# scroll-tech/halo2-snark-aggregator

Hardware: AMD Instinct MI355X
Metric: BN254 G1 MSM points/sec (higher is better)
Workload: dtype u32 (9 x 29-bit limbs, Montgomery R = 2^261; 254-bit prime-field integers)

## Files before the change

### halo2-snark-aggregator_amd/__init__.py

```python
from __future__ import annotations

import ctypes as C
import os
from typing import List, Optional, Sequence

_HERE = os.path.dirname(os.path.abspath(__file__))
LIB_PATH = os.path.join(_HERE, "libh2agg.so")
HEADER_PATH = os.path.join(os.path.dirname(_HERE), "include", "h2agg.h")

OK, ERR_INVALID, ERR_DIV_ZERO, ERR_EMPTY, ERR_HIP, ERR_NONCANONICAL, ERR_NOMEM, ERR_BAD_POINT, ERR_PEER, ERR_NOT_IN_TABLE = range(10)
OP_ADD, OP_SUB, OP_MUL, OP_SQR, OP_INV, OP_DIV = range(6)
FR_FFT_LOCAL = 10
FR_FFT_MAX_K = 24
FR_POLY_CHUNK = 11
FR_SCAN_CHUNK = 11
FR_PROD_MAX_COLUMNS = 16
FR_SORT_TILE = 11
FR_SORT_TILE_MIN = 4
FR_COMPRESS_MAX_COLUMNS = 1 << 16
EXPR_MAX_DEPTH = 16

IDENTITY_JAC = (0).to_bytes(32, "little") + (1).to_bytes(32, "little") + (0).to_bytes(32, "little")


# ... 21 lines not shown
def load_library():
    global _lib
    if _lib is not None:
        return _lib
    if not os.path.exists(LIB_PATH):
        raise ImportError(
            "libh2agg.so is not built (%s). Run `python __graft_entry__.py build` — the HIP extension is "
            "required, there is no CPU fallback." % LIB_PATH)
    try:
        import torch
    except ImportError:
        pass
    lib = C.CDLL(LIB_PATH)
    u8p, vp, sz, i32, u64 = C.c_char_p, C.c_void_p, C.c_size_t, C.c_int, C.c_uint64
    ctxp = C.c_void_p
    protos = {
        "h2agg_create": (i32, [i32, C.POINTER(ctxp)]),
        "h2agg_destroy": (None, [ctxp]),
        "h2agg_last_error": (C.c_char_p, [ctxp]),
        "h2agg_set_stream": (i32, [ctxp, vp]),
        "h2agg_synchronize": (i32, [ctxp]),
        "h2agg_describe": (C.c_char_p, [ctxp]),
        "h2agg_fr_batch_op": (i32, [ctxp, i32, u8p, u8p, sz, vp]),
        "h2agg_fr_batch_pow_constant": (i32, [ctxp, u8p, sz, u64, vp]),
        "h2agg_fr_tape_eval": (i32, [ctxp, u8p, sz, vp, sz, vp, sz, vp]),
        "h2agg_fr_mul_add_accumulate": (i32, [ctxp, u8p, sz, u8p, vp]),
        "h2agg_fr_sum_with_coeff_and_constant": (i32, [ctxp, u8p, u8p, sz, u8p, vp]),
        "h2agg_g1_batch_add": (i32, [ctxp, u8p, u8p, sz, i32, vp]),
        "h2agg_g1_batch_scalar_mul": (i32, [ctxp, u8p, u8p, sz, vp]),
        "h2agg_g1_batch_to_affine": (i32, [ctxp, u8p, sz, vp]),
        "h2agg_g1_sum": (i32, [ctxp, u8p, sz, vp]),
        "h2agg_g1_batch_decompress": (i32, [ctxp, u8p, sz, vp, vp]),
        "h2agg_g1_batch_compress": (i32, [ctxp, u8p, sz, vp]),
        "h2agg_g1_msm": (i32, [ctxp, vp, vp, sz, vp]),
        "h2agg_g1_msm_jac": (i32, [ctxp, vp, vp, sz, vp]),
        "h2agg_g1_msm_segmented": (i32, [ctxp, vp, vp, sz, C.POINTER(u64), sz, vp]),
        "h2agg_host_alloc": (i32, [ctxp, sz, C.POINTER(vp)]),
        "h2agg_host_free": (i32, [ctxp, vp]),
        "h2agg_eval_flat": (i32, [ctxp, u8p, u8p, u8p, sz, vp]),
        "h2agg_bases_upload": (i32, [ctxp, u8p, sz, C.POINTER(u64)]),
        "h2agg_bases_generate": (i32, [ctxp, vp, sz, C.POINTER(u64)]),
        "h2agg_bases_precompute": (i32, [ctxp, u64, i32]),
        "h2agg_bases_download": (i32, [ctxp, u64, sz, sz, vp]),
        "h2agg_bases_free": (i32, [ctxp, u64]),
        "h2agg_g1_msm_preloaded": (i32, [ctxp, u64, u8p, sz, vp]),
        "h2agg_instance_commitment": (i32, [ctxp, u64, u8p, sz, sz, vp]),
        "h2agg_g1_msm_device": (i32, [ctxp, u64, vp, sz, vp]),
        "h2agg_g1_msm_device_async": (i32, [ctxp, u64, vp, sz, vp]),
        "h2agg_schema_create": (i32, [ctxp, C.POINTER(C.c_void_p)]),
        "h2agg_schema_destroy": (None, [C.c_void_p]),
        "h2agg_schema_node_commitment": (i32, [C.c_void_p, C.c_char_p, u8p, C.POINTER(C.c_uint32)]),
        "h2agg_schema_node_eval": (i32, [C.c_void_p, u8p, C.POINTER(C.c_uint32)]),
        "h2agg_schema_node_scalar": (i32, [C.c_void_p, u8p, C.POINTER(C.c_uint32)]),
        "h2agg_schema_node_add": (i32, [C.c_void_p, C.c_uint32, C.c_uint32, C.POINTER(C.c_uint32)]),
        "h2agg_schema_node_mul": (i32, [C.c_void_p, C.c_uint32, C.c_uint32, C.POINTER(C.c_uint32)]),
        "h2agg_schema_estimate": (i32, [C.c_void_p, C.c_uint32, C.POINTER(C.c_size_t)]),
        "h2agg_schema_evaluation_queries": (i32, [C.c_void_p, sz, C.POINTER(C.c_char_p), u8p, u8p,
                                                  C.POINTER(C.c_uint32)]),
        "h2agg_schema_batch_multi_open": (i32, [C.c_void_p, C.c_char_p, sz, C.POINTER(C.c_int32), u8p,
                                                C.POINTER(C.c_uint32), sz, u8p, u8p, u8p,
                                                C.POINTER(C.c_uint32), C.POINTER(C.c_uint32)]),
        "h2agg_schema_eval": (i32, [C.c_void_p, C.c_uint32, vp, C.POINTER(i32), vp]),
        "h2agg_evaluate_multiopen_proof": (i32, [C.c_void_p, C.c_uint32, C.c_uint32, vp, vp]),
        "h2agg_evaluate_multiopen_prepare": (i32, [C.c_void_p, C.c_uint32, C.c_uint32]),
        "h2agg_schema_name_count": (C.c_size_t, [C.c_void_p]),
        "h2agg_schema_name": (C.c_char_p, [C.c_void_p, C.c_size_t]),
        "h2agg_g1_msm_device_batch_async": (C.c_int, [C.c_void_p, C.c_uint64, C.c_void_p, C.c_size_t, C.c_size_t, C.c_void_p]),
        "h2agg_schema_query_set_commitment": (C.c_int, [C.c_void_p, C.c_uint32, C.c_char_p]),
        "h2agg_g1_batch_to_affine_device": (C.c_int, [C.c_void_p, C.c_void_p, C.c_size_t, C.c_char_p]),
        "h2agg_schema_names_joined": (C.c_size_t, [C.c_void_p, C.c_char_p, C.c_size_t]),
        "h2agg_schema_point_list_len": (C.c_size_t, [C.c_void_p]),
        "h2agg_poseidon_squeeze_batch": (i32, [ctxp, u8p, sz, sz, C.POINTER(C.c_uint32), sz, vp]),
        "h2agg_transcript_read_batch": (i32, [ctxp, u8p, sz, sz, C.c_char_p, sz, u8p, sz, u8p, sz, vp, vp]),
        "h2agg_vk_create": (i32, [ctxp, u8p, sz, C.POINTER(C.c_void_p)]),
        "h2agg_vk_set_transcript": (i32, [C.c_void_p, i32]),
        "h2agg_hash_transcript_read_batch": (i32, [ctxp, i32, u8p, sz, sz, C.c_char_p, sz, u8p, sz, u8p, sz, vp, vp]),
        "h2agg_hash_transcript_read_batch_host": (i32, [i32, u8p, sz, sz, C.c_char_p, sz, u8p, sz, u8p, sz, vp, vp, i32]),
        "h2agg_hash_digest_host": (i32, [i32, u8p, sz, vp]),
        "h2agg_vk_destroy": (None, [C.c_void_p]),
        "h2agg_verify_aggregation": (i32, [ctxp, vp, sz, u8p, u8p, vp, vp, vp, C.POINTER(i32)]),
        "h2agg_verify_aggregation_ex": (i32, [ctxp, vp, sz, u8p, u8p, vp, vp, vp, C.POINTER(i32), vp, sz]),
        "h2agg_verify_aggregation_sharded": (i32, [ctxp, vp, sz, vp, u8p, u8p, vp, vp, vp, C.POINTER(i32), vp, sz]),
        "h2agg_debug_configure": (i32, [ctxp, C.c_char_p, i32]),
        "h2agg_verify_proofs": (i32, [ctxp, vp, sz, u8p, u8p, vp, vp, C.POINTER(C.c_int32), C.POINTER(i32), vp, sz]),
        "h2agg_verify_plan_stats": (i32, [ctxp, C.POINTER(C.c_uint64), C.POINTER(C.c_uint64), C.POINTER(C.c_uint64)]),
        "h2agg_last_phases": (C.c_char_p, [ctxp]),
        "h2agg_transcript_configure": (i32, [ctxp, i32]),
        "h2agg_poseidon_squeeze_batch_host": (i32, [u8p, sz, sz, C.POINTER(C.c_uint32), sz, vp, i32]),
        "h2agg_host_threads": (i32, []),
        "h2agg_host_sponge_kind": (i32, []),
        "h2agg_comm_unique_id": (i32, [vp]),
        "h2agg_comm_init_rank": (i32, [ctxp, u8p, i32, i32]),
        "h2agg_comm_create": (i32, [C.POINTER(i32), i32, C.POINTER(ctxp)]),
        "h2agg_comm_size": (i32, [ctxp]),
        "h2agg_comm_rank": (i32, [ctxp]),
        "h2agg_comm_last_error": (C.c_char_p, []),
        "h2agg_allgather_add_points": (i32, [C.POINTER(ctxp), i32, u8p, sz, vp]),
        "h2agg_pairing_check": (i32, [ctxp, u8p, u8p, sz, C.POINTER(i32)]),
        "h2agg_g2_batch_decompress": (i32, [ctxp, u8p, sz, vp]),
        "h2agg_bases_fft": (i32, [ctxp, u64, C.c_uint, i32, C.POINTER(u64)]),
        "h2agg_params_setup": (i32, [ctxp, C.c_uint, u8p, C.POINTER(u64), C.POINTER(u64)]),
        "h2agg_fr_fft": (i32, [ctxp, vp, C.c_uint, i32, u8p, vp]),
        "h2agg_fr_fft_device": (i32, [ctxp, vp, C.c_uint, i32, u8p, vp]),
        "h2agg_fr_poly_eval": (i32, [ctxp, vp, sz, C.c_uint, C.POINTER(C.c_uint32), sz, u8p, sz, vp]),
        "h2agg_fr_poly_eval_device": (i32, [ctxp, vp, sz, C.c_uint, C.POINTER(C.c_uint32), sz, u8p, sz, vp]),
        "h2agg_fr_poly_divide": (i32, [ctxp, vp, C.c_uint, u8p, vp, vp]),
        "h2agg_fr_poly_divide_device": (i32, [ctxp, vp, C.c_uint, u8p, vp, vp]),
        "h2agg_kzg_multiopen": (i32, [ctxp, u64, vp, sz, C.c_uint, C.POINTER(C.c_uint32), sz, u8p, sz, u8p, vp,
                                      C.POINTER(C.c_uint32), C.POINTER(sz)]),
        "h2agg_kzg_multiopen_device": (i32, [ctxp, u64, vp, sz, C.c_uint, C.POINTER(C.c_uint32), sz, u8p, sz, u8p, vp,
                                             C.POINTER(C.c_uint32), C.POINTER(sz)]),
        "h2agg_fr_batch_invert": (i32, [ctxp, vp, sz, vp]),
        "h2agg_fr_batch_invert_device": (i32, [ctxp, vp, sz, vp]),
        "h2agg_fr_grand_product": (i32, [ctxp, vp, vp, C.c_uint, sz, u8p, vp, vp]),
        "h2agg_fr_grand_product_device": (i32, [ctxp, vp, vp, C.c_uint, sz, u8p, vp, vp]),
        "h2agg_permutation_product": (i32, [ctxp, vp, vp, sz, C.c_uint, sz, u8p, u8p, u8p, u8p, u8p, vp, vp]),
        "h2agg_permutation_product_device": (i32, [ctxp, vp, vp, sz, C.c_uint, sz, u8p, u8p, u8p, u8p, u8p, vp, vp]),
        "h2agg_lookup_product": (i32, [ctxp, vp, vp, vp, vp, C.c_uint, sz, u8p, u8p, vp, vp]),
        "h2agg_lookup_product_device": (i32, [ctxp, vp, vp, vp, vp, C.c_uint, sz, u8p, u8p, vp, vp]),
        "h2agg_lookup_permute": (i32, [ctxp, vp, vp, C.c_uint, sz, vp, vp]),
        "h2agg_lookup_permute_device": (i32, [ctxp, vp, vp, C.c_uint, sz, vp, vp]),
        "h2agg_fr_columns_compress": (i32, [ctxp, vp, sz, C.c_uint, u8p, vp]),
        "h2agg_fr_columns_compress_device": (i32, [ctxp, vp, sz, C.c_uint, u8p, vp]),
        "h2agg_vk_expressions_eval": (i32, [ctxp, vp, i32, sz, C.c_uint, vp, vp, vp, u8p, u8p, vp]),
        "h2agg_vk_expressions_eval_device": (i32, [ctxp, vp, i32, sz, C.c_uint, vp, vp, vp, u8p, u8p, vp]),
        "h2agg_quotient": (i32, [ctxp, vp, vp, vp, vp, vp, vp, vp, vp, vp, u8p, u8p, u8p, u8p, u8p, u8p, vp]),
        "h2agg_quotient_device": (i32, [ctxp, vp, vp, vp, vp, vp, vp, vp, vp, vp, u8p, u8p, u8p, u8p, u8p, u8p, vp]),
        "h2agg_g2_scalar_mul": (i32, [u8p, u8p, vp]),
        "h2agg_g2_batch_compress": (i32, [u8p, sz, vp]),
        "h2agg_pairing_product": (i32, [ctxp, u8p, u8p, sz, vp]),
        "h2agg_final_pair_check": (i32, [ctxp, u8p, u8p, u8p, u8p, C.POINTER(i32)]),
        "h2agg_msm_configure": (i32, [ctxp, i32, i32, i32]),
        "h2agg_msm_configure_glv": (i32, [ctxp, i32]),
        "h2agg_msm_configure_lanes_per_bucket": (i32, [ctxp, i32]),
        "h2agg_msm_configure_sort": (i32, [ctxp, i32, i32]),
        "h2agg_msm_set_tail_overlap": (i32, [ctxp, i32]),
        "h2agg_profile_enable": (i32, [ctxp, i32]),
        "h2agg_profile_reset": (i32, [ctxp]),
        "h2agg_profile_stage_count": (i32, [ctxp]),
        "h2agg_profile_stage_name": (C.c_char_p, [ctxp, i32]),
        "h2agg_profile_stage_get": (i32, [ctxp, i32, C.POINTER(C.c_double), C.POINTER(u64)]),
    }
    for name, (res, args) in protos.items():
        fn = getattr(lib, name)
        fn.restype = res
        fn.argtypes = args
    lib._h2agg_protos = tuple(protos)
    _lib = lib
    return lib


def exported_symbols() -> Sequence[str]:
    return load_library()._h2agg_protos


def _need(buf, nbytes: int, what: str):
    if buf is None or len(buf) != nbytes:
        raise ValueError("%s must be exactly %d bytes (got %s)" % (what, nbytes, "None" if buf is None else len(buf)))


def _check_host(rc: int, what: str):
    if rc == ERR_BAD_POINT:
        raise BadPoint(rc, what + ": invalid G2 point")
    if rc != OK:
        raise H2AggError(rc, what + (": input integer >= modulus" if rc == ERR_NONCANONICAL else " failed"))

# ... 548 lines not shown
        self._check(self._lib.h2agg_hash_transcript_read_batch(self._ctx, *args, pts, ch))
        nproofs = len(proofs)
        return ([pts.raw[64 * npts * i:64 * npts * (i + 1)] for i in range(nproofs)],
                [ch.raw[32 * nsq * i:32 * nsq * (i + 1)] for i in range(nproofs)])

    @staticmethod
    def comm_unique_id() -> bytes:
        out = C.create_string_buffer(128)
        rc = load_library().h2agg_comm_unique_id(out)
        if rc != OK:
            why = load_library().h2agg_comm_last_error() or b""
            raise H2AggError(rc, "h2agg_comm_unique_id failed: " + (why.decode(errors="replace") or "RCCL error"))
        return out.raw

    def comm_init_rank(self, unique_id: bytes, rank: int, nranks: int):
        _need(unique_id, 128, "unique_id")
        self._check(self._lib.h2agg_comm_init_rank(self._ctx, unique_id, rank, nranks))

    def comm_size(self) -> int:
        return self._lib.h2agg_comm_size(self._ctx)

    def comm_rank(self) -> int:
        return self._lib.h2agg_comm_rank(self._ctx)

    def allgather_add_points(self, partial_jac: bytes) -> bytes:
        npts = len(partial_jac) // 96
        _need(partial_jac, 96 * npts, "partial_jac")
        out = C.create_string_buffer(max(64 * npts, 1))
        arr = (C.c_void_p * 1)(self._ctx)
        self._check(self._lib.h2agg_allgather_add_points(arr, 1, partial_jac, npts, out))
        return out.raw[:64 * npts]

    def pairing_check(self, g1_aff: bytes, g2_aff: bytes) -> bool:
        n = len(g1_aff) // 64
        _need(g1_aff, 64 * n, "g1_aff")
        _need(g2_aff, 128 * n, "g2_aff")
        ok = C.c_int()
        self._check(self._lib.h2agg_pairing_check(self._ctx, g1_aff, g2_aff, n, C.byref(ok)))
        return bool(ok.value)

    def pairing_product(self, g1_aff: bytes, g2_aff: bytes) -> bytes:
        n = len(g1_aff) // 64
        _need(g1_aff, 64 * n, "g1_aff")
        _need(g2_aff, 128 * n, "g2_aff")
        out = C.create_string_buffer(384)
        self._check(self._lib.h2agg_pairing_product(self._ctx, g1_aff, g2_aff, n, out))
        return out.raw

    def g2_batch_decompress(self, data: bytes) -> bytes:
        n = len(data) // 64
        _need(data, 64 * n, "data")
        out = C.create_string_buffer(max(128 * n, 1))
        self._check(self._lib.h2agg_g2_batch_decompress(self._ctx, data, n, out))
        return out.raw[:128 * n]

    def final_pair_check(self, left_aff: bytes, right_aff: bytes, s_g2: bytes, g2: bytes) -> bool:
        _need(left_aff, 64, "left_aff")
        _need(right_aff, 64, "right_aff")
        _need(s_g2, 128, "s_g2")
        _need(g2, 128, "g2")
        ok = C.c_int()
        self._check(self._lib.h2agg_final_pair_check(self._ctx, left_aff, right_aff, s_g2, g2, C.byref(ok)))
        return bool(ok.value)

    def g1_msm_device_batch_async(self, handle: int, d_scalars_ptr: int, n: int, batch: int, d_out_ptr: int):
        self._check(self._lib.h2agg_g1_msm_device_batch_async(self._ctx, handle, C.c_void_p(d_scalars_ptr), n, batch,
                                                              C.c_void_p(d_out_ptr)))

    def msm_configure(self, window_bits: int = 0, reduce_segment: int = 0, big_bucket_threshold: int = 0):
        self._check(self._lib.h2agg_msm_configure(self._ctx, window_bits, reduce_segment, big_bucket_threshold))

    def msm_configure_glv(self, mode: int = 0):
        self._check(self._lib.h2agg_msm_configure_glv(self._ctx, mode))

    def msm_configure_lanes_per_bucket(self, lanes: int = 0):
        self._check(self._lib.h2agg_msm_configure_lanes_per_bucket(self._ctx, lanes))

    def msm_configure_sort(self, sub_bits: int = 0, tile: int = 0):
        self._check(self._lib.h2agg_msm_configure_sort(self._ctx, sub_bits, tile))

    def debug_configure(self, key: str, value: int):
        self._check(self._lib.h2agg_debug_configure(self._ctx, key.encode(), int(value)))

    def msm_set_tail_overlap(self, level: int = 2):
        self._check(self._lib.h2agg_msm_set_tail_overlap(self._ctx, int(level)))

    def profile_enable(self, on=True, only_stage: Optional[int] = None):
        mode = (2 + int(only_stage)) if (on and only_stage is not None) else int(bool(on))
        self._check(self._lib.h2agg_profile_enable(self._ctx, mode))

    def profile_reset(self):
        self._check(self._lib.h2agg_profile_reset(self._ctx))

    def profile_stages(self):
        out = {}
        for i in range(self._lib.h2agg_profile_stage_count(self._ctx)):
            ms, cnt = C.c_double(), C.c_uint64()
            self._check(self._lib.h2agg_profile_stage_get(self._ctx, i, C.byref(ms), C.byref(cnt)))
            out[self._lib.h2agg_profile_stage_name(self._ctx, i).decode()] = (ms.value, cnt.value)
        return out


def host_sponge_kind() -> str:
    return "ifma" if load_library().h2agg_host_sponge_kind() == 1 else "scalar"


def poseidon_squeeze_batch_host(elems: bytes, nproofs: int, upto: Sequence[int], max_threads: int = 0,
                                kernel: Optional[str] = None) -> bytes:
    lib = load_library()
    max_threads = (max_threads & 0xffff) | {None: 0, "scalar": 0x10000, "ifma": 0x20000}[kernel]
    nelem = (len(elems) // 32) // max(nproofs, 1)
    _need(elems, 32 * nelem * nproofs, "elems")
    nsq = len(upto)
    arr = (C.c_uint32 * max(nsq, 1))(*upto)
    out = C.create_string_buffer(32 * max(nproofs * nsq, 1))
    rc = lib.h2agg_poseidon_squeeze_batch_host(elems, nproofs, nelem, arr, nsq, out, max_threads)
    if rc != OK:
        raise H2AggError(rc, "h2agg_poseidon_squeeze_batch_host: " + ("element >= r" if rc == ERR_NONCANONICAL else "invalid arguments"))
    return out.raw[:32 * nproofs * nsq]


TRANSCRIPT_KINDS = {"poseidon": 0, "sha256": 1, "keccak256": 2}


def _hash_transcript_args(kind, proofs, script, consts, ext_points_aff):
    nproofs = len(proofs)
    plen = 64 * script.count("P") + 32 * script.count("S")
    for p in proofs:
        _need(p, plen, "proof")
    npts, nsq, nx = script.count("P"), script.count("Q"), script.count("X")
    _need(consts, 32 * script.count("C"), "consts")
    _need(ext_points_aff, 64 * nx * nproofs, "ext_points_aff")
    pts = C.create_string_buffer(max(64 * npts * nproofs, 1))
    ch = C.create_string_buffer(max(32 * nsq * nproofs, 1))
    sb = script.encode()
    k = TRANSCRIPT_KINDS.get(kind, kind)
    return (k, b"".join(proofs), plen, nproofs, sb, len(sb), consts, len(consts) // 32, ext_points_aff, nx), pts, ch, npts, nsq


def hash_transcript_read_batch_host(kind: str, proofs: Sequence[bytes], script: str, consts: bytes = b"",
                                    ext_points_aff: bytes = b"", max_threads: int = 0):
    args, pts, ch, npts, nsq = _hash_transcript_args(kind, proofs, script, consts, ext_points_aff)
    rc = load_library().h2agg_hash_transcript_read_batch_host(*args, pts, ch, max_threads)
    if rc != OK:
        what = {ERR_BAD_POINT: "invalid point encoding in proof", ERR_NONCANONICAL: "invalid field element encoding in proof"}
        raise (BadPoint if rc == ERR_BAD_POINT else H2AggError)(rc, "h2agg_hash_transcript_read_batch_host: " + what.get(rc, "invalid arguments"))
    nproofs = len(proofs)
    return ([pts.raw[64 * npts * i:64 * npts * (i + 1)] for i in range(nproofs)],
            [ch.raw[32 * nsq * i:32 * nsq * (i + 1)] for i in range(nproofs)])


def hash_digest_host(kind: str, msg: bytes) -> bytes:
    out = C.create_string_buffer(32)
    rc = load_library().h2agg_hash_digest_host(TRANSCRIPT_KINDS.get(kind, kind), msg, len(msg), out)
    if rc != OK:
        raise H2AggError(rc, "h2agg_hash_digest_host: invalid arguments")
    return out.raw


def host_threads() -> int:
    return load_library().h2agg_host_threads()


class H2AggGroup:

    def __init__(self, devices: Sequence[int]):
# ... 156 lines not shown
```

### halo2-snark-aggregator_amd/csrc/batch_kernels.hpp

```cpp
#pragma once
#include "g1.hpp"

namespace h2agg {

enum : uint32_t { FLAG_NONCANONICAL = 1u, FLAG_DIV_ZERO = 2u, FLAG_BAD_POINT = 4u };

constexpr int BLOCK = 256;

__global__ void k_flags_roll(uint32_t* flags) {
    flags[2] |= flags[0];
    flags[0] = 0;
}

template <int NLIMB>
FP_INLINE void lds_put(uint32_t* lds, int tid, const uint32_t* v) {
#pragma unroll
    for (int k = 0; k < NLIMB; ++k) lds[k * BLOCK + tid] = v[k];
}
template <int NLIMB>
FP_INLINE void lds_get(const uint32_t* lds, int tid, uint32_t* v) {
#pragma unroll
    for (int k = 0; k < NLIMB; ++k) v[k] = lds[k * BLOCK + tid];
}
constexpr int XYZZ_WORDS = 4 * NL;
FP_INLINE void lds_put_xyzz(uint32_t* lds, int tid, const G1XYZZ& p) {
    lds_put<NL>(lds, tid, p.x.l);
    lds_put<NL>(lds + NL * BLOCK, tid, p.y.l);
    lds_put<NL>(lds + 2 * NL * BLOCK, tid, p.zz.l);
    lds_put<NL>(lds + 3 * NL * BLOCK, tid, p.zzz.l);
}
FP_INLINE G1XYZZ lds_get_xyzz(const uint32_t* lds, int tid) {
    G1XYZZ p;
    lds_get<NL>(lds, tid, p.x.l);
    lds_get<NL>(lds + NL * BLOCK, tid, p.y.l);
    lds_get<NL>(lds + 2 * NL * BLOCK, tid, p.zz.l);
    lds_get<NL>(lds + 3 * NL * BLOCK, tid, p.zzz.l);
    return p;
}
__device__ __noinline__ G1XYZZ block_sum_xyzz(G1XYZZ v, uint32_t* lds) {
    const int tid = threadIdx.x;
    lds_put_xyzz(lds, tid, v);
    __syncthreads();
#pragma unroll 1
    for (int s = BLOCK / 2; s >= 1; s >>= 1) {
        if (tid < s) {
            G1XYZZ o = lds_get_xyzz(lds, tid + s);
            v = xyzz_add(v, o);
            lds_put_xyzz(lds, tid, v);
        }
        __syncthreads();
    }
    return v;
}
__device__ __noinline__ Fr block_sum_fr(Fr v, uint32_t* lds) {
    const int tid = threadIdx.x;
    lds_put<NL>(lds, tid, v.l);
    __syncthreads();
#pragma unroll 1
    for (int s = BLOCK / 2; s >= 1; s >>= 1) {
        if (tid < s) {
            Fr o;
            lds_get<NL>(lds, tid + s, o.l);
            v = fp_cond_sub<FrParams>(fp_add<FrParams>(v, o));
            lds_put<NL>(lds, tid, v.l);
        }
        __syncthreads();
    }
    return v;
}

__global__ void __launch_bounds__(BLOCK) k_fr_batch_op(int op, const uint8_t* __restrict__ a,
                                                       const uint8_t* __restrict__ b, size_t n,
                                                       uint8_t* __restrict__ out, uint32_t* flags) {
    for (size_t i = (size_t)blockIdx.x * BLOCK + threadIdx.x; i < n; i += (size_t)gridDim.x * BLOCK) {
        Fr x = fp_load<FrParams>(a + 32 * i);
        uint32_t bad = !fp_is_canonical<FrParams>(x);
        Fr y = Fr::zero();
        if (op <= 2 || op == 5) {
            y = fp_load<FrParams>(b + 32 * i);
            bad |= !fp_is_canonical<FrParams>(y);
        }
        if (bad) atomicOr(flags, FLAG_NONCANONICAL);
        Fr z;
        switch (op) {
        case 0: z = fp_cond_sub<FrParams>(fp_add<FrParams>(x, y)); break;
        case 1: z = fp_cond_sub<FrParams>(fp_sub<1, FrParams>(x, y)); break;
        case 2: z = fp_cond_sub<FrParams>(fp_mul<FrParams>(fp_to_mont<FrParams>(x), y)); break;
        case 3: z = fp_cond_sub<FrParams>(fp_mul<FrParams>(fp_to_mont<FrParams>(x), x)); break;
        case 5:
            if (y.is_zero_int()) atomicOr(flags, FLAG_DIV_ZERO);
            z = fp_cond_sub<FrParams>(fp_mul<FrParams>(fp_inv<FrParams>(fp_to_mont<FrParams>(y)), x));
            break;
        default:
            if (x.is_zero_int()) atomicOr(flags, FLAG_DIV_ZERO);
            z = fp_from_mont<FrParams>(fp_inv<FrParams>(fp_to_mont<FrParams>(x)));
// ... 124 lines not shown
__device__ __noinline__ G1XYZZ g1_scalar_mul(const G1Affine& base, const U256& s) {
    G1XYZZ acc = G1XYZZ::identity();
    U256 k = s;
#pragma unroll 1
    for (int it = 0; it < 256; ++it) {
        acc = xyzz_double(acc);
        const uint32_t top = k.w[7] >> 31;
#pragma unroll
        for (int i = 7; i > 0; --i) k.w[i] = (k.w[i] << 1) | (k.w[i - 1] >> 31);
        k.w[0] <<= 1;
        if (top) xyzz_add_affine(acc, base);
    }
    return acc;
}

__global__ void __launch_bounds__(BLOCK) k_g1_batch_scalar_mul(const uint8_t* __restrict__ bases,
                                                               const uint8_t* __restrict__ scalars, size_t n,
                                                               uint8_t* __restrict__ out, uint32_t* flags) {
    for (size_t i = (size_t)blockIdx.x * BLOCK + threadIdx.x; i < n; i += (size_t)gridDim.x * BLOCK) {
        uint32_t bad = 0;
        G1Affine p = affine_load_canonical(bases + 64 * i, bad);
        U256 s = u256_load(scalars + 32 * i);
        bad |= !u256_is_canonical_fr(s);
        if (bad) atomicOr(flags, FLAG_NONCANONICAL);
        jac_store_canonical(out + 96 * i, jac_from_xyzz(g1_scalar_mul(p, s)));
    }
}

FP_INLINE G1Affine affine_from_xyzz(const G1XYZZ& p) {
    G1Affine r;
    if (p.is_identity()) {
        r.x = Fq::zero();
        r.y = Fq::zero();
        return r;
    }
    Fq i = fp_inv<FqParams>(FQ_MUL(p.zz, p.zzz));
    r.x = FQ_MUL(p.x, FQ_MUL(i, p.zzz));
    r.y = FQ_MUL(p.y, FQ_MUL(i, p.zz));
    return r;
}

constexpr int TA_K = 8;
template <bool MONT>
FP_INLINE void jac_batch_normalise(const uint8_t* __restrict__ in, size_t n, uint8_t* __restrict__ out, uint32_t* flags) {
    const size_t stride = (size_t)gridDim.x * BLOCK;
    for (size_t i0 = (size_t)blockIdx.x * BLOCK + threadIdx.x; i0 < n; i0 += stride * TA_K) {
        Fq pre[TA_K];
        Fq run = Fq::one();
        uint32_t bad = 0;
#pragma unroll
        for (int j = 0; j < TA_K; ++j) {
            const size_t i = i0 + (size_t)j * stride;
            Fq z = Fq::one();
            if (i < n) {
                bad |= jac_noncanonical(in + 96 * i);
                const Fq zc = fp_to_mont<FqParams>(fp_load<FqParams>(in + 96 * i + 64));
                if (!fp_is_zero_mod<2, FqParams>(zc)) z = zc;
            }
            pre[j] = run;
            run = FQ_MUL(run, z);
        }
        if (bad) atomicOr(flags, FLAG_NONCANONICAL);
        Fq inv = fp_inv<FqParams>(run);
#pragma unroll
        for (int j = TA_K - 1; j >= 0; --j) {
            const size_t i = i0 + (size_t)j * stride;
            if (i >= n) continue;
            const Fq zc = fp_to_mont<FqParams>(fp_load<FqParams>(in + 96 * i + 64));
            const bool ident = fp_is_zero_mod<2, FqParams>(zc);
            Fq ox = Fq::zero(), oy = Fq::zero();
            if (!ident) {
                const Fq zi = FQ_MUL(inv, pre[j]);
                inv = FQ_MUL(inv, zc);
                const Fq zi2 = FQ_SQR(zi);
                const Fq x = fp_to_mont<FqParams>(fp_load<FqParams>(in + 96 * i));
                const Fq y = fp_to_mont<FqParams>(fp_load<FqParams>(in + 96 * i + 32));
                ox = FQ_MUL(x, zi2);
                oy = FQ_MUL(y, FQ_MUL(zi2, zi));
                if (!MONT) {
                    ox = fp_from_mont<FqParams>(ox);
                    oy = fp_from_mont<FqParams>(oy);
                }
            }
            fp_store<FqParams>(out + 64 * i, ox);
            fp_store<FqParams>(out + 64 * i + 32, oy);
        }
    }
}
__global__ void __launch_bounds__(BLOCK) k_g1_batch_to_affine(const uint8_t* __restrict__ in, size_t n,
                                                              uint8_t* __restrict__ out, uint32_t* flags) {
    jac_batch_normalise<false>(in, n, out, flags);
}
__global__ void __launch_bounds__(BLOCK) k_jac_to_mont_affine(const uint8_t* __restrict__ in, size_t n,
                                                              uint8_t* __restrict__ out, uint32_t* flags) {
    jac_batch_normalise<true>(in, n, out, flags);
}

FP_INLINE Fq fq_sqrt_candidate(const Fq& a) {
    constexpr uint32_t E[8] = {0xb61f3f52u, 0x4f082305u, 0x5a1c72a3u, 0x65e05aa4u,
                               0xa0605617u, 0x6e14116du, 0xb84c680au, 0x0c19139cu};
    Fq acc = Fq::one();
#pragma unroll 1
    for (int bit = 251; bit >= 0; --bit) {
        acc = FQ_SQR(acc);
        uint32_t w = 0;
#pragma unroll
        for (int i = 0; i < 8; ++i) w = (bit / 32 == i) ? E[i] : w;
        if ((w >> (bit % 32)) & 1u) acc = FQ_MUL(acc, a);
    }
    return acc;
}
FP_INLINE bool g1_decompress_one(U256 w, Fq& ox, Fq& oy) {
    const uint32_t ysign = w.w[7] >> 31;
    w.w[7] &= 0x7fffffffu;
    Fq x = fp_unpack<FqParams>(w.w);
    bool good = fp_is_canonical<FqParams>(x);
    ox = Fq::zero();
    oy = Fq::zero();
    if (good && !(x.is_zero_int() && !ysign)) {
        const Fq xm = fp_to_mont<FqParams>(x);
        Fq three;
#pragma unroll
        for (int k = 0; k < NL; ++k) three.l[k] = 0;
        three.l[0] = 3;
        const Fq rhs = FQ_ADD(FQ_MUL(FQ_SQR(xm), xm), fp_to_mont<FqParams>(three));
        const Fq y = fq_sqrt_candidate(rhs);
        good = fp_is_zero_mod<8, FqParams>(FQ_SUB(4, FQ_SQR(y), rhs));
        Fq yc = fp_from_mont<FqParams>(y);
        if ((yc.l[0] & 1u) != ysign) {
            int32_t d[NL];
#pragma unroll
            for (int k = 0; k < NL; ++k) d[k] = (int32_t)FqParams::MOD[k] - (int32_t)yc.l[k];
            yc = fp_normalize<FqParams>(d);
        }
        if (good) {
            ox = x;
            oy = yc;
        }
    }
    return good;
}
__global__ void __launch_bounds__(BLOCK) k_g1_batch_decompress(const uint8_t* __restrict__ in, size_t n,
                                                               uint8_t* __restrict__ out_aff, uint8_t* __restrict__ ok,
                                                               uint32_t* flags) {
    for (size_t i = (size_t)blockIdx.x * BLOCK + threadIdx.x; i < n; i += (size_t)gridDim.x * BLOCK) {
        Fq ox, oy;
        const bool good = g1_decompress_one(u256_load(in + 32 * i), ox, oy);
        if (!good) atomicOr(flags, FLAG_BAD_POINT);
        if (ok) ok[i] = good ? 1 : 0;
        fp_store<FqParams>(out_aff + 64 * i, ox);
        fp_store<FqParams>(out_aff + 64 * i + 32, oy);
    }
}
__global__ void __launch_bounds__(BLOCK) k_g1_batch_compress(const uint8_t* __restrict__ aff, size_t n,
                                                             uint8_t* __restrict__ out, uint32_t* flags) {
    for (size_t i = (size_t)blockIdx.x * BLOCK + threadIdx.x; i < n; i += (size_t)gridDim.x * BLOCK) {
        Fq x = fp_load<FqParams>(aff + 64 * i), y = fp_load<FqParams>(aff + 64 * i + 32);
        if (!fp_is_canonical<FqParams>(x) | !fp_is_canonical<FqParams>(y)) atomicOr(flags, FLAG_NONCANONICAL);
        uint32_t w[8];
        fp_pack<FqParams>(w, x);
        if (!(x.is_zero_int() && y.is_zero_int())) w[7] |= (y.l[0] & 1u) << 31;
        uint4* o = reinterpret_cast<uint4*>(out + 32 * i);
        o[0] = make_uint4(w[0], w[1], w[2], w[3]);
        o[1] = make_uint4(w[4], w[5], w[6], w[7]);
    }
}

__global__ void __launch_bounds__(BLOCK) k_g1_sum(const uint8_t* __restrict__ in, size_t n, uint8_t* __restrict__ out,
                                                  uint32_t* flags) {
    __shared__ uint32_t lds[XYZZ_WORDS * BLOCK];
    G1XYZZ acc = G1XYZZ::identity();
    for (size_t i = threadIdx.x; i < n; i += BLOCK) {
        if (jac_noncanonical(in + 96 * i)) atomicOr(flags, FLAG_NONCANONICAL);
        acc = xyzz_add(acc, xyzz_from_jac(jac_load_canonical(in + 96 * i)));
    }
    G1XYZZ tot = block_sum_xyzz(acc, lds);
    if (threadIdx.x == 0) jac_store_canonical(out, jac_from_xyzz(tot));
}

FP_INLINE bool jac_on_curve(const G1Jac& p) {
    if (fp_is_zero_mod<2, FqParams>(p.z)) return true;
    Fq three;
#pragma unroll
    for (int k = 0; k < NL; ++k) three.l[k] = 0;
    three.l[0] = 3;
    const Fq z2 = FQ_SQR(p.z);
    const Fq z6 = FQ_MUL(FQ_SQR(z2), z2);
    const Fq rhs = FQ_ADD(FQ_MUL(FQ_SQR(p.x), p.x), FQ_MUL(z6, fp_to_mont<FqParams>(three)));
    return fp_is_zero_mod<8, FqParams>(FQ_SUB(4, FQ_SQR(p.y), rhs));
}

__global__ void __launch_bounds__(BLOCK) k_g1_sum_strided_affine(const uint8_t* __restrict__ in, size_t world, size_t npts,
                                                                 uint8_t* __restrict__ out_aff, uint32_t* flags) {
    __shared__ uint32_t lds[XYZZ_WORDS * BLOCK];
    const size_t k = blockIdx.x;
    G1XYZZ acc = G1XYZZ::identity();
    for (size_t r = threadIdx.x; r < world; r += BLOCK) {
        const uint8_t* p = in + 96 * (r * npts + k);
        if (jac_noncanonical(p)) atomicOr(flags, FLAG_NONCANONICAL);
        const G1Jac j = jac_load_canonical(p);
        if (!jac_on_curve(j)) atomicOr(flags, FLAG_BAD_POINT);
        acc = xyzz_add(acc, xyzz_from_jac(j));
    }
    G1XYZZ tot = block_sum_xyzz(acc, lds);
    if (threadIdx.x == 0) {
        const G1Affine a = affine_from_xyzz(tot);
        fp_store<FqParams>(out_aff + 64 * k, fp_from_mont<FqParams>(a.x));
        fp_store<FqParams>(out_aff + 64 * k + 32, fp_from_mont<FqParams>(a.y));
    }
}

__global__ void __launch_bounds__(BLOCK) k_bases_to_mont(const uint8_t* __restrict__ in, size_t n,
                                                         uint8_t* __restrict__ out, uint32_t* flags) {
    for (size_t i = (size_t)blockIdx.x * BLOCK + threadIdx.x; i < n; i += (size_t)gridDim.x * BLOCK) {
        uint32_t bad = 0;
        G1Affine p = affine_load_canonical(in + 64 * i, bad);
        if (bad) atomicOr(flags, FLAG_NONCANONICAL);
        affine_store(out + 64 * i, p);
    }
}
__global__ void __launch_bounds__(BLOCK) k_bases_from_mont(const uint8_t* __restrict__ in, size_t n,
                                                           uint8_t* __restrict__ out) {
    for (size_t i = (size_t)blockIdx.x * BLOCK + threadIdx.x; i < n; i += (size_t)gridDim.x * BLOCK) {
        G1Affine p = affine_load(in + 64 * i);
        fp_store<FqParams>(out + 64 * i, fp_from_mont<FqParams>(p.x));
        fp_store<FqParams>(out + 64 * i + 32, fp_from_mont<FqParams>(p.y));
    }
}
__global__ void __launch_bounds__(BLOCK) k_bases_generate(const uint8_t* __restrict__ k, size_t n,
                                                          uint8_t* __restrict__ out, uint32_t* flags) {
    for (size_t i = (size_t)blockIdx.x * BLOCK + threadIdx.x; i < n; i += (size_t)gridDim.x * BLOCK) {
        U256 s = u256_load(k + 32 * i);
        if (!u256_is_canonical_fr(s)) atomicOr(flags, FLAG_NONCANONICAL);
        G1Affine g;
        g.x = Fq::one();
        g.y = FQ_DBL(Fq::one());
        affine_store(out + 64 * i, affine_from_xyzz(g1_scalar_mul(g, s)));
    }
}

}
```

### halo2-snark-aggregator_amd/csrc/fp.hpp

```cpp
#pragma once
#include <hip/hip_runtime.h>
#include <stdint.h>

#define FP_INLINE __device__ __forceinline__

namespace h2agg {

constexpr int NL = 9;
constexpr uint32_t M29 = (1u << 29) - 1u;

struct FqParams {
    static constexpr uint32_t MOD[9] = {0x187cfd47u, 0x010460b6u, 0x1c72a34fu, 0x02d522d0u, 0x1585d978u,
                                        0x02db40c0u, 0x00a6e141u, 0x0e5c2634u, 0x0030644eu};
    static constexpr uint32_t NINV = 0x04866389u;
    static constexpr uint32_t R1[9] = {0x157ccc21u, 0x141c2758u, 0x185230d3u, 0x014c0419u, 0x0aa36fb9u,
                                       0x1d4240ceu, 0x11d54c07u, 0x052ac7a8u, 0x000dc836u};
    static constexpr uint32_t R2[9] = {0x059bac10u, 0x0d1503a3u, 0x018016b8u, 0x10ab0ca8u, 0x02632639u,
                                       0x02c0169fu, 0x169bfd53u, 0x11869d4cu, 0x002a11a6u};
};
struct FrParams {
    static constexpr uint32_t MOD[9] = {0x10000001u, 0x1f0fac9fu, 0x0e5c2450u, 0x07d090f3u, 0x1585d283u,
                                        0x02db40c0u, 0x00a6e141u, 0x0e5c2634u, 0x0030644eu};
    static constexpr uint32_t NINV = 0x0fffffffu;
    static constexpr uint32_t R1[9] = {0x0fffff57u, 0x1ea70ab4u, 0x052c068bu, 0x17504f49u, 0x0aa8075bu,
// ... 11 lines not shown
        out = (j < 8) ? (uint32_t)(t & M29) : (uint32_t)t;
        c = t >> 29;
    }
    return out;
}

template <class P>
struct Fp {
    uint32_t l[NL];

    static FP_INLINE Fp zero() {
        Fp r;
#pragma unroll
        for (int i = 0; i < NL; ++i) r.l[i] = 0;
        return r;
    }
    static FP_INLINE Fp one() {
        Fp r;
#pragma unroll
        for (int i = 0; i < NL; ++i) r.l[i] = P::R1[i];
        return r;
    }
    static FP_INLINE Fp r2() {
        Fp r;
#pragma unroll
        for (int i = 0; i < NL; ++i) r.l[i] = P::R2[i];
        return r;
    }
    FP_INLINE bool is_zero_int() const {
        uint32_t o = 0;
#pragma unroll
        for (int i = 0; i < NL; ++i) o |= l[i];
        return o == 0;
    }
    FP_INLINE bool same_int(const Fp& b) const {
        uint32_t o = 0;
#pragma unroll
        for (int i = 0; i < NL; ++i) o |= (l[i] ^ b.l[i]);
        return o == 0;
    }
};

template <class P>
FP_INLINE Fp<P> fp_normalize(const int32_t (&x)[NL]) {
    Fp<P> r;
    int32_t c = 0;
#pragma unroll
    for (int i = 0; i < 8; ++i) {
        int32_t t = x[i] + c;
        r.l[i] = (uint32_t)t & M29;
        c = t >> 29;
    }
    r.l[8] = (uint32_t)(x[8] + c);
    return r;
}

template <class P>
FP_INLINE Fp<P> fp_add(const Fp<P>& a, const Fp<P>& b) {
    int32_t x[NL];
#pragma unroll
    for (int i = 0; i < NL; ++i) x[i] = (int32_t)(a.l[i] + b.l[i]);
    return fp_normalize<P>(x);
}
template <class P>
FP_INLINE Fp<P> fp_dbl(const Fp<P>& a) {
    int32_t x[NL];
#pragma unroll
    for (int i = 0; i < NL; ++i) x[i] = (int32_t)(a.l[i] << 1);
    return fp_normalize<P>(x);
}
template <int K, class P>
FP_INLINE Fp<P> fp_sub(const Fp<P>& a, const Fp<P>& b) {
    int32_t x[NL];
#pragma unroll
    for (int i = 0; i < NL; ++i) x[i] = (int32_t)(a.l[i] + km_limb<P>(K, i)) - (int32_t)b.l[i];
    return fp_normalize<P>(x);
}
template <int K, class P>
FP_INLINE Fp<P> fp_neg(const Fp<P>& a) {
    int32_t x[NL];
#pragma unroll
    for (int i = 0; i < NL; ++i) x[i] = (int32_t)km_limb<P>(K, i) - (int32_t)a.l[i];
    return fp_normalize<P>(x);
}

template <class P>
FP_INLINE Fp<P> fp_mont_reduce(uint64_t (&acc)[18]) {
#pragma unroll
    for (int k = 0; k < NL; ++k) {
        const uint32_t m = ((uint32_t)acc[k] * P::NINV) & M29;
#pragma unroll
        for (int j = 0; j < NL; ++j) acc[k + j] += (uint64_t)m * P::MOD[j];
        acc[k + 1] += acc[k] >> 29;
    }
    Fp<P> r;
    uint64_t c = 0;
#pragma unroll
    for (int i = 0; i < 8; ++i) {
        uint64_t t = acc[9 + i] + c;
        r.l[i] = (uint32_t)t & M29;
        c = t >> 29;
    }
    r.l[8] = (uint32_t)(acc[17] + c);
    return r;
}

template <class P, class ColF>
FP_INLINE Fp<P> fp_mont_ps(ColF&& col) {
    uint32_t m[NL];
    Fp<P> r;
    uint64_t t = 0, u = 0;
#pragma unroll
    for (int k = 0; k < NL; ++k) {
        col(k, t, u);
#pragma unroll
        for (int i = 0; i < k; ++i) {
            if (i & 1) t += (uint64_t)m[i] * P::MOD[k - i];
            else u += (uint64_t)m[i] * P::MOD[k - i];
        }
        t += u;
        u = 0;
        m[k] = ((uint32_t)t * P::NINV) & M29;
        t += (uint64_t)m[k] * P::MOD[0];
        t >>= 29;
    }
#pragma unroll
    for (int k = NL; k < 2 * NL - 1; ++k) {
        col(k, t, u);
#pragma unroll
        for (int i = k - (NL - 1); i < NL; ++i) {
            if (i & 1) t += (uint64_t)m[i] * P::MOD[k - i];
            else u += (uint64_t)m[i] * P::MOD[k - i];
        }
        t += u;
        u = 0;
        r.l[k - NL] = (uint32_t)t & M29;
        t >>= 29;
    }
    r.l[NL - 1] = (uint32_t)t;
    return r;
}
template <class P>
FP_INLINE void fp_col_mul(int k, const Fp<P>& a, const Fp<P>& b, uint64_t& t, uint64_t& u) {
#pragma unroll
    for (int i = 0; i < NL; ++i) {
        const int j = k - i;
        if (j >= 0 && j < NL) {
            if (i & 1) u += (uint64_t)a.l[i] * b.l[j];
            else t += (uint64_t)a.l[i] * b.l[j];
        }
    }
}
template <class P>
FP_INLINE Fp<P> fp_mul_ps(const Fp<P>& a, const Fp<P>& b) {
    return fp_mont_ps<P>([&](int k, uint64_t& t, uint64_t& u) { fp_col_mul<P>(k, a, b, t, u); });
}
template <class P>
FP_INLINE Fp<P> fp_mul2_ps(const Fp<P>& a, const Fp<P>& b, const Fp<P>& c, const Fp<P>& d) {
    return fp_mont_ps<P>([&](int k, uint64_t& t, uint64_t& u) {
        fp_col_mul<P>(k, a, b, t, u);
        fp_col_mul<P>(k, c, d, u, t);
    });
}
template <class P>
FP_INLINE Fp<P> fp_mul3_ps(const Fp<P>& a, const Fp<P>& b, const Fp<P>& c, const Fp<P>& d, const Fp<P>& e, const Fp<P>& f) {
    return fp_mont_ps<P>([&](int k, uint64_t& t, uint64_t& u) {
// ... 454 lines not shown
```

### halo2-snark-aggregator_amd/csrc/h2agg.hip

```cpp
#include "../../include/h2agg.h"

#include <hip/hip_runtime.h>

#include <chrono>
#include <cstdlib>
#include <cstdio>
#include <cstring>
#include <algorithm>
#include <csignal>
#include <dlfcn.h>
#include <unistd.h>
#include <atomic>
#include <condition_variable>
#include <functional>
#include <mutex>
#include <thread>
#include <sched.h>
#include <sys/resource.h>
#include <map>
#include <memory>
#include <new>
#include <string>
#include <vector>

#include "scalar_mul_kernels.hpp"
#include "lp_kernels.hpp"
#include "seg_msm_kernels.hpp"
#include "g1_fft_kernels.hpp"
#include "fr_fft_kernels.hpp"
#include "poly_kernels.hpp"
#include "prod_kernels.hpp"
#include "lookup_kernels.hpp"
#include "quotient_kernels.hpp"
#include "pairing.hpp"
#if !defined(__HIP_DEVICE_COMPILE__) && defined(__x86_64__)
#define H2AGG_PAIRING_ADX_BUILD 1
#define PAIRING_NS pairing_adx
#define PAIRING_ADX 1
#pragma clang attribute push(__attribute__((target("bmi2,adx"))), apply_to = function)
#include "pairing.hpp"
#pragma clang attribute pop
#undef PAIRING_NS
#undef PAIRING_ADX
#endif
#include "poseidon_host.hpp"
#include "poseidon_sponge_host.hpp"
#include "poseidon_ifma_host.hpp"
#include "poseidon_kernels.hpp"
#include "hash_transcript_host.hpp"
#include "hash_transcript_kernels.hpp"

using namespace h2agg;

namespace {

#ifdef H2AGG_MEASURE_KNOBS
static inline const char* knob(const char* name) { return getenv(name); }
#else
static inline const char* knob(const char*) { return nullptr; }
#endif
static const bool ev_scope_system = knob("H2AGG_EVENT_SCOPE") && !strcmp(knob("H2AGG_EVENT_SCOPE"), "system");
#define EV_SYNC_FLAGS (ev_scope_system ? hipEventDisableTiming : (hipEventDisableTiming | hipEventReleaseToDevice))
#define EV_TIME_FLAGS (ev_scope_system ? hipEventDefault : hipEventReleaseToDevice)

struct DevBuf {
    void* p = nullptr;
    size_t cap = 0;
};

enum Stage {
    ST_PART_COUNT = 0, ST_PART_SCATTER, ST_BUCKET_SORT, ST_ORDER, ST_ACCUM, ST_ACCUM_BIG, ST_REDUCE, ST_WINDOW_SUM,
    ST_FINAL, ST_N
};
const char* const STAGE_NAMES[ST_N] = {"msm_part_count", "msm_part_scatter",   "msm_bucket_sort",
                                       "msm_order",      "msm_accumulate",     "msm_accumulate_big",
                                       "msm_reduce",     "msm_window_sum",     "msm_final"};

struct Table {
    uint8_t* d = nullptr;
    uint8_t* endo_x = nullptr;
    size_t n = 0;
    uint8_t* pre = nullptr;
    int pre_c = 0, pre_W = 0;
    uint8_t* comb = nullptr;
    size_t comb_n = 0;
    std::vector<uint8_t*> comb_retired;
    void free_combs() {
        if (comb) hipFree(comb);
        for (uint8_t* p : comb_retired) hipFree(p);
        comb = nullptr;
        comb_n = 0;
        comb_retired.clear();
    }
};
struct PreTable {
    const uint8_t* d;
    size_t n_level;
    int c, W;
};

}

constexpr int MSM_MAX_SLICES = 16;
enum { CHAIN_OFF = 0, CHAIN_FIRST = 1, CHAIN_MID = 2, CHAIN_LAST = 3 };

struct h2agg_ctx {
    int device = 0;
    hipStream_t own_stream = nullptr;
    hipStream_t stream = nullptr;
    std::string err;
    std::string desc;
    int cu_count = 0;

    DevBuf in_a, in_b, in_c, out, tmp_bases;
    DevBuf comb;
    bool comb_ready = false;
    DevBuf psd_spec, tr_in, tr_points, tr_elems, tr_chal;
    bool psd_ready = false;
    int cfg_transcript = 0;
    std::vector<uint8_t> h_elems;
    DevBuf inst_vals, inst_jac, inst_aff, agg_elems;
    DevBuf hist[2], offs[2], pmeta[2], order[2], entries[2];
    DevBuf big_list[2], big_keys[2], big_part[2];
    DevBuf fix_list[2];
    bool meta_clean[2] = {};
    DevBuf item_idx, item_sub,
        glv_buf, parts, small, endo_buf, tile_counts, fb_long;
    uint32_t* d_flags = nullptr;
    uint8_t* d_res_xyzz = nullptr;
    uint8_t* d_res_jac = nullptr;
    uint8_t* h_pinned = nullptr;

    DevBuf sch_regs, sch_in, sch_scalars[2], sch_bases[2], sch_endo;
    uint8_t* h_stage = nullptr;
    size_t h_stage_cap = 0;
    uint8_t* h_down = nullptr;
    size_t h_down_cap = 0;
    const void* sch_owner = nullptr;
    struct AggPlanCache* agg_plans = nullptr;

    hipStream_t copy_stream = nullptr;
    hipStream_t spare_streams[4] = {};
    hipStream_t aux_stream = nullptr;
    hipEvent_t ev_aux = nullptr, ev_aux_go = nullptr;
    hipEvent_t ev_copy[MSM_MAX_SLICES] = {}, ev_copy_s[MSM_MAX_SLICES] = {}, ev_ready = nullptr;

    std::map<uint64_t, Table> tables;
    uint64_t next_handle = 1;

    void* comm = nullptr;
    int comm_rank = 0, comm_size = 0;

    int dbg_pcie_slices = 0, dbg_pcie_glv = 0, dbg_pcie_chain = 1, dbg_comb_msm = 1, dbg_plan_cache = 1, dbg_small_sort = 1, dbg_eval_split = 1, dbg_pre_big = 0, dbg_lean_acc = 1, dbg_shard_fail = 0, dbg_shard_calls = 0, dbg_phases = 0, dbg_tape_lds = 1, dbg_prewake = 1;
    int dbg_seg_chunk = 0, dbg_seg_c = 0;
    DevBuf seg_wsum, seg_dev, seg_out;
    DevBuf fft_tw[2], fft_scale;
    int fft_tw_k[2] = {-1, -1};
    bool fft_scale_ready = false;
    DevBuf frfft_tw[2], frfft_shift, frfft_work;
    int frfft_tw_k[2] = {-1, -1};
    int dbg_fr_fft_local = 0;
    DevBuf poly_work, poly_desc, poly_slab, poly_jac;
    int dbg_fr_poly_chunk = 0;
    DevBuf prod_num, prod_den, prod_lvl, prod_tab;
    int dbg_fr_scan_chunk = 0;
    DevBuf lk_work, lk_desc;
    int dbg_fr_sort_tile = 0;
    DevBuf qt_work, qt_prog, qt_tab;
    std::string last_phases;
    int cfg_c = 0, cfg_seg = 0, cfg_big = 0, cfg_sub_bits = 0, cfg_tile = 0;
    int cfg_glv = 0;
    int cfg_lpb = 0;
    bool cfg_no_stage = false, cfg_stage_l1 = false, staged_attr_set = false, cfg_no_dm = false, dm_attr_set = false, r2d_attr_set = false;

    bool tail_overlap = false;
    int overlap_level = 2;
    static constexpr int TAIL_SLOTS = 3;
    DevBuf r2d_ticket[TAIL_SLOTS];
    DevBuf buckets[TAIL_SLOTS], segsum[TAIL_SLOTS], wsum[TAIL_SLOTS];
    hipStream_t tail_streams[TAIL_SLOTS] = {};
    hipEvent_t ev_bulk[TAIL_SLOTS] = {}, ev_tail[TAIL_SLOTS] = {};
    bool tail_pending[TAIL_SLOTS] = {};
    int parity = 0;
    int chain = 0;
    size_t chain_n = 0;
    bool chain_glv = false;
    std::function<int(hipStream_t)> bases_hook;
    std::function<int(bool)> deferred_tail;
    hipEvent_t ev_sortdone = nullptr;
    hipStream_t acc_stream = nullptr;
    hipEvent_t ev_sorted[2] = {}, ev_accdone[2] = {};
    bool accdone_pending[2] = {};
    int sort_par = 0;

    static constexpr int PROF_RING = 32;
    struct ProfSlot {
        hipEvent_t ev[ST_N][2] = {};
        bool used[ST_N] = {};
        bool pending = false;
    };
    bool profiling = false;
    int prof_only = -1;
    bool prof_events_created = false;
    ProfSlot prof[PROF_RING];
    int prof_cur = 0;
    double stage_ms[ST_N] = {};
    uint64_t stage_launches[ST_N] = {};
};

namespace {

int fail(h2agg_ctx* c, int code, const std::string& msg) {
    if (c) c->err = msg;
    return code;
}

#define HIP_TRY(ctx, expr)                                                                              \
    do {                                                                                                \
        hipError_t e_ = (expr);                                                                         \
        if (e_ != hipSuccess)                                                                           \
            return fail(ctx, H2AGG_ERR_HIP, std::string(#expr) + ": " + hipGetErrorString(e_));         \
    } while (0)

int flush_deferred_tail(h2agg_ctx* c, bool behind_sort);

int ensure(h2agg_ctx* c, DevBuf& b, size_t bytes) {
    if (bytes <= b.cap) return H2AGG_OK;
    if (b.p) {
        {
            const int rc_ = flush_deferred_tail(c, false);
            if (rc_ != H2AGG_OK) return rc_;
        }
        HIP_TRY(c, hipDeviceSynchronize());
        HIP_TRY(c, hipFree(b.p));
    }
    b.p = nullptr;
    b.cap = 0;
    size_t want = bytes + bytes / 8 + 256;
    hipError_t e = hipMalloc(&b.p, want);
    if (e != hipSuccess) return fail(c, H2AGG_ERR_NOMEM, std::string("hipMalloc: ") + hipGetErrorString(e));
    b.cap = want;
    return H2AGG_OK;
}

#define TRY(expr)                      \
    do {                               \
        int rc_ = (expr);              \
        if (rc_ != H2AGG_OK) return rc_; \
    } while (0)

int grid_for(const h2agg_ctx* c, size_t n) {
    size_t blocks = (n + BLOCK - 1) / BLOCK;
    size_t cap = (size_t)c->cu_count * 8;
    if (blocks > cap) blocks = cap;
    if (blocks < 1) blocks = 1;
    return (int)blocks;
}

int clear_flags(h2agg_ctx* c) {
    hipLaunchKernelGGL(k_flags_roll, dim3(1), dim3(1), 0, c->stream, c->d_flags);
    return H2AGG_OK;
}

int flags_to_status(h2agg_ctx* c, uint32_t f, bool earlier) {
    const char* pre = earlier ? "an earlier asynchronous call on this context: " : "";
    if (f & FLAG_DIV_ZERO)
        return fail(c, H2AGG_ERR_DIV_ZERO, std::string(pre) + "inversion of zero (reference: invert().unwrap() panics)");
    if (f & FLAG_NONCANONICAL) return fail(c, H2AGG_ERR_NONCANONICAL, std::string(pre) + "input integer >= modulus");
    if (f & FLAG_BAD_POINT) return fail(c, H2AGG_ERR_BAD_POINT, std::string(pre) + "invalid point encoding in proof");
    if (f & FLAG_NOT_IN_TABLE) return fail(c, H2AGG_ERR_NOT_IN_TABLE, std::string(pre) + "a lookup input does not occur in the table");
    return H2AGG_OK;
}

int finish(h2agg_ctx* c, uint32_t host_flags = 0) {
    HIP_TRY(c, hipMemcpyAsync(c->h_pinned + 2048, c->d_flags, 12, hipMemcpyDeviceToHost, c->stream));
    HIP_TRY(c, hipStreamSynchronize(c->stream));
    uint32_t f[3];
    memcpy(f, c->h_pinned + 2048, 12);
    f[0] |= host_flags;
    if (f[0] | f[2]) HIP_TRY(c, hipMemsetAsync(c->d_flags, 0, 12, c->stream));
    if (f[0]) return flags_to_status(c, f[0], false);
    return flags_to_status(c, f[2], true);
}

int window_count(int c, bool glv) { return glv ? (128 + c - 1) / c : (255 + c - 1) / c; }
int top_window_bits(int c, bool glv) { return (glv ? 127 : 254) - c * (window_count(c, glv) - 1); }
int choose_window(size_t n, bool glv) {
    if (glv) return n <= ((size_t)1 << 12) ? 8 : n <= ((size_t)1 << 14) ? 13 : 16;
    return n <= ((size_t)1 << 12) ? 8 : n < ((size_t)1 << 19) ? 15 : n < ((size_t)3 << 19) ? 16 : 17;
}

MsmPlan make_plan(const h2agg_ctx* c, size_t n, uint32_t batch = 1) {
    MsmPlan p;
    p.glv = c->cfg_glv > 0 ||
            (c->cfg_glv == 0 && !(c->tail_overlap && n >= ((size_t)1 << 20)) && n < ((size_t)1 << 22));
    p.c = c->cfg_c ? c->cfg_c : choose_window(n, p.glv);
    p.W = window_count(p.c, p.glv);
    p.NB = 1u << (p.c - 1);
    p.NBT = (uint32_t)p.W * batch * p.NB;
    uint32_t seg = c->cfg_seg ? (uint32_t)c->cfg_seg
                              : (p.NBT >= (1u << 18) ? (c->tail_overlap && p.NBT >= (1u << 19) ? 32u : 8u)
                                                     : (p.NBT >= (1u << 15) ? 4u : 2u));
    if (seg > p.NB) seg = p.NB;
    p.seg = seg;
    p.spw = p.NB / seg;
    p.big = c->cfg_big ? (uint32_t)c->cfg_big : 256u;
    return p;
}

struct StageTimer {
    h2agg_ctx* c;
    int st;
    hipStream_t s;
    StageTimer(h2agg_ctx* c_, int st_, hipStream_t s_ = nullptr) : c(c_), st(st_), s(s_ ? s_ : c_->stream) {
        if (c->profiling && (c->prof_only < 0 || c->prof_only == st)) {
            hipEventRecord(c->prof[c->prof_cur].ev[st][0], s);
        }
    }
    ~StageTimer() {
        if (c->profiling && (c->prof_only < 0 || c->prof_only == st)) {
            hipEventRecord(c->prof[c->prof_cur].ev[st][1], s);
            c->prof[c->prof_cur].used[st] = true;
        }
    }
};

struct Crumbs {
    static constexpr int N = 48;
    std::atomic<uint32_t> at{0};
    uintptr_t addr[N] = {};
    uint64_t note[N] = {};
    bool on = false;
};
Crumbs g_crumbs;
void crumbs_dump(int) {
    Dl_info info;
    uintptr_t base = 0;
    if (dladdr((void*)&crumbs_dump, &info)) base = (uintptr_t)info.dli_fbase;
    const uint32_t end = g_crumbs.at.load();
    fprintf(stderr, "[h2agg breadcrumbs pid %d] last entries, oldest first (addresses relative to libh2agg.so):\n", (int)getpid());
    for (uint32_t k = end > Crumbs::N ? end - Crumbs::N : 0; k < end; ++k)
        fprintf(stderr, "  #%u  +0x%zx  note %llu\n", k, (size_t)(g_crumbs.addr[k % Crumbs::N] - base), (unsigned long long)g_crumbs.note[k % Crumbs::N]);
    fflush(stderr);
    signal(SIGABRT, SIG_DFL);
    abort();
}
inline void crumb(uintptr_t a, uint64_t note) {
    if (!g_crumbs.on) return;
    const uint32_t k = g_crumbs.at.fetch_add(1) % Crumbs::N;
    g_crumbs.addr[k] = a;
    g_crumbs.note[k] = note;
}
struct CrumbsInit {
    CrumbsInit() {
        if (knob("H2AGG_BREADCRUMBS")) {
            g_crumbs.on = true;
            signal(SIGABRT, crumbs_dump);
        }
    }
} g_crumbs_init;

// ... 50 lines not shown
        fprintf(stderr, "[h2agg] streams that hold the main stream up when busy:");
        for (int i = 0; i < np; ++i) fprintf(stderr, " %d%s", i, blocks[i] ? "*" : "");
        fprintf(stderr, "  (* = shares its queue)\n");
    }
    if (nfree < h2agg_ctx::TAIL_SLOTS + 2) return H2AGG_OK;
    hipStream_t ordered[NP];
    int no = 0;
    for (int i = 0; i < np; ++i)
        if (!blocks[i]) ordered[no++] = pool[i];
    for (int i = 0; i < np; ++i)
        if (blocks[i]) ordered[no++] = pool[i];
    int at = 0;
    for (int k = 0; k < h2agg_ctx::TAIL_SLOTS; ++k) c->tail_streams[k] = ordered[at++];
    c->aux_stream = ordered[at++];
    c->copy_stream = ordered[at++];
    c->acc_stream = ordered[at++];
    for (int k = 0; k < 4; ++k) c->spare_streams[k] = ordered[at++];
    return H2AGG_OK;
}

void profile_harvest(h2agg_ctx* c, int slot) {
    h2agg_ctx::ProfSlot& ps = c->prof[slot];
    if (!ps.pending) return;
    for (int s = 0; s < ST_N; ++s) {
        if (!ps.used[s]) continue;
        float ms = 0.f;
        hipEventSynchronize(ps.ev[s][1]);
        if (hipEventElapsedTime(&ms, ps.ev[s][0], ps.ev[s][1]) == hipSuccess) {
            c->stage_ms[s] += ms;
            c->stage_launches[s] += 1;
        }
        ps.used[s] = false;
    }
    ps.pending = false;
}
void profile_begin_call(h2agg_ctx* c) {
    if (!c->profiling) return;
    profile_harvest(c, c->prof_cur);
}
void profile_end_call(h2agg_ctx* c) {
    if (!c->profiling) return;
    c->prof[c->prof_cur].pending = true;
    c->prof_cur = (c->prof_cur + 1) % h2agg_ctx::PROF_RING;
}
void profile_harvest_all(h2agg_ctx* c) {
    for (int k = 0; k < h2agg_ctx::PROF_RING; ++k) profile_harvest(c, k);
}

int flush_deferred_tail(h2agg_ctx* c, bool behind_sort) {
    if (!c->deferred_tail) return H2AGG_OK;
    std::function<int(bool)> f;
    f.swap(c->deferred_tail);
    return f(behind_sort);
}

int join_tails(h2agg_ctx* c) {
    TRY(flush_deferred_tail(c, false));
    for (int k = 0; k < h2agg_ctx::TAIL_SLOTS; ++k) {
        if (c->tail_pending[k]) {
            HIP_TRY(c, hipStreamWaitEvent(c->stream, c->ev_tail[k], 0));
            c->tail_pending[k] = false;
        }
    }
    for (int q = 0; q < 2; ++q) {
        if (c->accdone_pending[q]) {
            HIP_TRY(c, hipStreamWaitEvent(c->stream, c->ev_accdone[q], 0));
            c->accdone_pending[q] = false;
        }
    }
    return H2AGG_OK;
}

bool msm_split_ok(const h2agg_ctx* c, size_t n_total) {
    if (!c->dbg_small_sort || n_total < 2 || n_total > (size_t)SMALL_SORT_N) return false;
    if (c->cfg_no_stage || c->cfg_stage_l1 || c->cfg_sub_bits || c->cfg_tile || c->chain) return false;
    const MsmPlan p = make_plan(c, n_total, 2);
    return p.NB <= (uint32_t)SMALL_SORT_NB;
}

bool fb_sort_knobs_clear(const h2agg_ctx* c) {
    return !c->cfg_no_dm && !c->cfg_no_stage && !c->cfg_stage_l1 && !c->cfg_sub_bits && !c->cfg_tile && !c->cfg_seg;
}

int msm_run(h2agg_ctx* c, const uint8_t* d_bases, const uint8_t* d_scalars, size_t n_base, uint8_t* d_out_jac,
            uint32_t batch = 1, const uint8_t* d_endo_x = nullptr, const PreTable* pre = nullptr, uint32_t split = 0) {
    if (split) batch = 2;
    const size_t n = split ? n_base : n_base * batch;
    crumb((uintptr_t)__builtin_return_address(0), ((uint64_t)batch << 40) | n_base);
    if (n >= ((size_t)1 << 30)) return fail(c, H2AGG_ERR_INVALID, "n must be < 2^30");
    const int chain = (pre || batch != 1) ? CHAIN_OFF : c->chain;
    MsmPlan p = make_plan(c, chain ? c->chain_n : n_base, batch);
    if (chain && p.glv != c->chain_glv) {
        const int was = c->cfg_glv;
        c->cfg_glv = c->chain_glv ? 1 : -1;
        p = make_plan(c, c->chain_n, batch);
        c->cfg_glv = was;
    }
    int Wd = p.W;
    const bool fbdm = pre && batch == 1 && pre->c == FB_C && pre->W == FB_W && pre->n_level <= ((size_t)FB_MAX_TILES * FB_T) &&
                      fb_sort_knobs_clear(c);
    const uint32_t fb_ntile = (uint32_t)((n + FB_T - 1) / FB_T);
    if (pre) {
        p.glv = false;
        p.c = pre->c;
        Wd = pre->W;
        p.W = 1;
        p.NB = 1u << (p.c - 1);
        p.NBT = fbdm ? FB_NBT : batch * p.NB;
        p.seg = c->cfg_seg ? (uint32_t)c->cfg_seg : (batch >= 16 ? 32u : 16u);
        if (p.seg > p.NB) p.seg = p.NB;
        p.spw = p.NB / p.seg;
        d_bases = pre->d;
    }
    const int W1 = p.W;
    const uint32_t WT = (uint32_t)W1 * batch;
    const size_t nent = n * (size_t)Wd * (p.glv ? 2 : 1);
    if (!c->cfg_big) {
        const size_t mean = nent / p.NBT;
        if (8 * mean > p.big) p.big = (uint32_t)(8 * mean);
    }
    if (nent >= ((size_t)1 << 32)) return fail(c, H2AGG_ERR_INVALID, "n * windows must be < 2^32");
    SortPlan sp;
    int want_sub = c->cfg_sub_bits ? c->cfg_sub_bits : SORT_SUB_BITS;
    if (pre && !c->cfg_sub_bits) {
        while (want_sub > 4 && (((size_t)p.NB * batch) >> want_sub) < 256) --want_sub;
    }
    sp.sub_bits = (p.c - 1 < want_sub) ? p.c - 1 : want_sub;
    while ((WT * (p.NB >> sp.sub_bits)) > (uint32_t)SORT_MAX_PW && sp.sub_bits < p.c - 1 &&
           sp.sub_bits < SORT_MAX_SUB_BITS)
        ++sp.sub_bits;
    sp.SB = 1u << sp.sub_bits;
    sp.ppw = p.NB >> sp.sub_bits;
    sp.PW = WT * sp.ppw;
    if (batch > 1 && !split) {
        sp.n_base = (uint32_t)n_base;
        sp.W1 = (uint32_t)W1;
    }
    if (pre) sp.pre_n = (uint32_t)pre->n_level;
    sp.tile = c->cfg_tile ? (uint32_t)c->cfg_tile : 2048u;
    sp.glv = p.glv;
    const int idx_bits = (p.glv ? 30 : 31) - sp.sub_bits;
    bool staged = !c->cfg_no_stage && (pre ? (size_t)pre->W * pre->n_level : n_base) <= ((size_t)1 << idx_bits);
    const size_t keys_per_scalar = (size_t)Wd * (p.glv ? 2 : 1);
    if (staged && c->cfg_stage_l1 && (size_t)sp.tile * keys_per_scalar > (size_t)STAGE_ITEMS_L1)
        sp.tile = (uint32_t)(STAGE_ITEMS_L1 / keys_per_scalar);
    if (staged && sp.tile < (uint32_t)BLOCK) staged = false;
    if (sp.PW > (uint32_t)SORT_MAX_PW) return fail(c, H2AGG_ERR_INVALID, "too many sort partitions");
    const uint32_t nseg_total = WT * p.spw;
    static const int par4_env = knob("H2AGG_PAR4") ? atoi(knob("H2AGG_PAR4")) : 0;
    const bool par4 = par4_env ? par4_env > 0 : nseg_total <= (split ? 32768u : 16384u);
    constexpr uint32_t META_PW = DM_MAX_PW;
    constexpr uint32_t M_PSTART = META_PW + 64, M_PCURSOR = M_PSTART + META_PW + 64,
                       M_BCOUNT = M_PCURSOR + META_PW + 64, M_BSTART = M_BCOUNT + SIZE_BINS + 64,
                       M_BCURSOR = M_BSTART + SIZE_BINS + 64, M_BIG = M_BCURSOR + SIZE_BINS + 64, M_WORDS = M_BIG + 64;
    const bool piped = c->tail_overlap && c->overlap_level >= 3;
    const bool altbuf = c->tail_overlap && c->overlap_level >= 2;
    const int sq = altbuf ? c->sort_par : 0;
    {
        const size_t cap0 = c->pmeta[sq].cap;
        TRY(ensure(c, c->pmeta[sq], M_WORDS * 4));
        if (c->pmeta[sq].cap != cap0) c->meta_clean[sq] = false;
    }
    TRY(ensure(c, c->hist[sq], (size_t)p.NBT * 4));
    TRY(ensure(c, c->offs[sq], (size_t)p.NBT * 4));
    TRY(ensure(c, c->order[sq], (size_t)p.NBT * 4));
    static const bool dm_env_off = knob("H2AGG_SORT") && !strcmp(knob("H2AGG_SORT"), "packed");
    const size_t dm_row = p.glv ? 2 * n : n;
    const bool dm17 = p.c == 17 && !p.glv;
// ... 181 lines not shown
                hipLaunchKernelGGL(k_part_scatter_staged, dim3(ntiles), dim3(BLOCK), lds1, st, d_scalars, n, p.c, Wd,
                                   sp, idx_bits, pcursor, item_idx);
            else
                hipLaunchKernelGGL(k_part_scatter_packed, dim3(ntiles), dim3(BLOCK), 0, st, d_scalars, n, p.c, Wd, sp,
                                   idx_bits, pcursor, item_idx, (const uint32_t*)tile_counts);
        }
        {
            StageTimer t(c, ST_BUCKET_SORT);
            hipLaunchKernelGGL(k_bucket_sort_staged<SORT2_TB>, dim3(sp.PW), dim3(SORT2_TB), lds2, st, pstart, item_idx, sp, idx_bits,
                               p.NB, hist, offs, entries);
        }
    } else {
        {
            StageTimer t(c, ST_PART_SCATTER);
            hipLaunchKernelGGL(k_part_scatter, dim3(ntiles), dim3(BLOCK), 0, st, d_scalars, n, p.c, Wd, sp, pcursor,
                               item_idx, item_sub);
        }
        {
            StageTimer t(c, ST_BUCKET_SORT);
            hipLaunchKernelGGL(k_bucket_sort, dim3(sp.PW), dim3(BLOCK), 0, st, pstart, item_idx, item_sub, sp, p.NB,
                               hist, offs, entries);
        }
    }
    }
    const bool ordered = nent >= ((size_t)1 << 16);
    if (ordered) {
        StageTimer t(c, ST_ORDER);
        unsigned g = (p.NBT + BLOCK * 8 - 1) / (BLOCK * 8);
        if (g > (unsigned)c->cu_count * 4) g = (unsigned)c->cu_count * 4;
        hipLaunchKernelGGL(k_size_count, dim3(g), dim3(BLOCK), 0, st, hist, p.NBT, bin_count);
        hipLaunchKernelGGL(k_scan_small, dim3(1), dim3(BLOCK), 0, st, bin_count, (uint32_t)SIZE_BINS, bin_start,
                           bin_cursor);
        hipLaunchKernelGGL(k_size_scatter, dim3(g), dim3(BLOCK), 0, st, hist, p.NBT, bin_cursor, order);
    }
    if (c->deferred_tail) {
        HIP_TRY(c, hipEventRecord(c->ev_sortdone, st));
        TRY(flush_deferred_tail(c, true));
    }
    if (piped) {
        HIP_TRY(c, hipEventRecord(c->ev_sorted[sq], st));
        HIP_TRY(c, hipStreamWaitEvent(c->acc_stream, c->ev_sorted[sq], 0));
        st = c->acc_stream;
    }
    if (c->tail_pending[par]) {
        HIP_TRY(c, hipStreamWaitEvent(st, c->ev_tail[par], 0));
        c->tail_pending[par] = false;
    }
    uint32_t lpb = 1;
    if (c->cfg_lpb) lpb = (uint32_t)c->cfg_lpb;
    else
        while (lpb < 8 && (size_t)p.NBT * lpb < (size_t)8192 * 64 &&
               (chain ? c->chain_n * (size_t)Wd * (p.glv ? 2 : 1) : nent) >= (size_t)lpb * p.NBT)
            lpb *= 2;
    if (c->bases_hook) {
        TRY(c->bases_hook(st));
        if (endo_late)
            hipLaunchKernelGGL(k_bases_endo_x, dim3(grid_for(c, n_base)), dim3(BLOCK), 0, st, d_bases, n_base, (uint8_t*)c->endo_buf.p);
    }
    uint8_t* acc_out = buckets;
    if (lpb > 1) {
        TRY(ensure(c, c->parts, (size_t)p.NBT * lpb * XYZZ_BYTES));
        acc_out = (uint8_t*)c->parts.p;
    }
    static const int acc_block = knob("H2AGG_ACC_BLOCK") ? atoi(knob("H2AGG_ACC_BLOCK")) : 64;
#ifdef H2AGG_MEASURE_KNOBS
    static const bool lean_env = !(knob("H2AGG_ACC") && !strcmp(knob("H2AGG_ACC"), "generic"));
    const bool lean = lean_env && c->dbg_lean_acc;
#else
    const bool lean = true;
#endif
    uint32_t* fix_list = nullptr;
    if (lean) {
        TRY(ensure(c, c->fix_list[sq], (size_t)p.NBT * lpb * 8));
        fix_list = (uint32_t*)c->fix_list[sq].p;
    }
    debug_sync(2);
    chaos_wait(2, st);
    {
        StageTimer t(c, ST_ACCUM, st);
        static const int acc_lds = knob("H2AGG_ACC_LDS") ? atoi(knob("H2AGG_ACC_LDS")) : 0;
        if (lean) {
#ifdef H2AGG_MEASURE_KNOBS
            static const bool lean_dual = !(knob("H2AGG_ACC") && !strcmp(knob("H2AGG_ACC"), "lean1"));
            auto kacc = lean_dual ? (chain == CHAIN_FIRST ? k_msm_accumulate_lean<1, true> : (chain == CHAIN_MID || chain == CHAIN_LAST) ? k_msm_accumulate_lean<2, true> : k_msm_accumulate_lean<0, true>)
                                  : (chain == CHAIN_FIRST ? k_msm_accumulate_lean<1, false> : (chain == CHAIN_MID || chain == CHAIN_LAST) ? k_msm_accumulate_lean<2, false> : k_msm_accumulate_lean<0, false>);
#else
            auto kacc = chain == CHAIN_FIRST ? k_msm_accumulate_lean<1, true> : (chain == CHAIN_MID || chain == CHAIN_LAST) ? k_msm_accumulate_lean<2, true> : k_msm_accumulate_lean<0, true>;
#endif
            hipLaunchKernelGGL(kacc, dim3((unsigned)(((size_t)p.NBT * lpb + 63) / 64)), dim3(64), (size_t)acc_lds,
                               st, d_bases, d_endo_x, entries, offs, hist, ordered ? order : (uint32_t*)nullptr, p.NBT, p.big, lpb, acc_out,
                               big_list, big_keys, big_count, fix_list);
        } else {
#ifdef H2AGG_MEASURE_KNOBS
        auto kacc = chain == CHAIN_FIRST ? k_msm_accumulate<1> : (chain == CHAIN_MID || chain == CHAIN_LAST) ? k_msm_accumulate<2> : k_msm_accumulate<0>;
        hipLaunchKernelGGL(kacc, dim3((unsigned)(((size_t)p.NBT * lpb + acc_block - 1) / acc_block)), dim3(acc_block), (size_t)acc_lds,
                           st, d_bases, d_endo_x, entries, offs, hist, ordered ? order : (uint32_t*)nullptr, p.NBT, p.big, lpb, acc_out,
                           big_list, big_keys, big_count);
#endif
        }
    }
    const bool tail_big = altbuf && c->overlap_level >= 2 && lpb == 1 && (chain == CHAIN_OFF || chain == CHAIN_LAST) && !split;
    const uint32_t resume = (chain == CHAIN_MID || chain == CHAIN_LAST) ? 1u : 0u;
    const bool chain_open = chain == CHAIN_FIRST || chain == CHAIN_MID;
    const bool big_possible = nent / WT > p.big;
    auto big_kernels = [=](hipStream_t bs) {
        StageTimer t(c, ST_ACCUM_BIG, bs);
        if (lean)
            hipLaunchKernelGGL(k_msm_accumulate_fix, dim3((unsigned)std::min<size_t>((size_t)c->cu_count * 12, ((size_t)p.NBT * lpb + 63) / 64)), dim3(64), 0, bs, d_bases, d_endo_x, entries, offs,
                               hist, lpb, acc_out, (const uint32_t*)big_count, (const uint32_t*)fix_list);
        if (!big_possible && lpb == 1) return;
        size_t grid = max_slots;
        const size_t cap = (size_t)c->cu_count * 8;
        if (grid > cap) grid = cap;
        hipLaunchKernelGGL(k_msm_accumulate_big, dim3((unsigned)grid), dim3(64), 0, bs, d_bases, d_endo_x, entries, offs, hist,
                           acc_out, lpb, big_part, big_list, big_count, resume);
        size_t gk = max_keys < cap ? max_keys : cap;
        hipLaunchKernelGGL(k_msm_big_combine, dim3((unsigned)gk), dim3(64), 0, bs, big_part, big_keys, big_count,
                           acc_out, lpb, resume);
        if (lpb > 1 && !chain_open) {
            const uint32_t cbig = chain ? 0xffffffffu : p.big;
            const unsigned gq = (unsigned)(((size_t)p.NBT * 2 * lpb + BLOCK - 1) / BLOCK);
            if (p.NBT > 16384u || (lpb != 2 && lpb != 4 && lpb != 8))
                hipLaunchKernelGGL(k_msm_bucket_combine, dim3((p.NBT + BLOCK - 1) / BLOCK), dim3(BLOCK), 0, bs,
                                   (const uint8_t*)acc_out, hist, p.NBT, cbig, lpb, buckets);
            else if (lpb == 8)
                hipLaunchKernelGGL(k_msm_bucket_combine_par4<8>, dim3(gq), dim3(BLOCK), 0, bs, (const uint8_t*)acc_out, hist, p.NBT, cbig, buckets);
            else if (lpb == 4)
                hipLaunchKernelGGL(k_msm_bucket_combine_par4<4>, dim3(gq), dim3(BLOCK), 0, bs, (const uint8_t*)acc_out, hist, p.NBT, cbig, buckets);
            else
                hipLaunchKernelGGL(k_msm_bucket_combine_par4<2>, dim3(gq), dim3(BLOCK), 0, bs, (const uint8_t*)acc_out, hist, p.NBT, cbig, buckets);
        }
    };
    if (!tail_big) {
        big_kernels(st);
        if (altbuf) {
            HIP_TRY(c, hipEventRecord(c->ev_accdone[sq], st));
            c->accdone_pending[sq] = true;
        }
    }
    if (altbuf) c->sort_par ^= 1;
    if (chain_open) {
        HIP_TRY(c, hipGetLastError());
        profile_end_call(c);
        return H2AGG_OK;
    }
#ifdef H2AGG_MEASURE_KNOBS
    static const int dbg_skip = knob("H2AGG_DBG_SKIP") ? atoi(knob("H2AGG_DBG_SKIP")) : 0;
#else
    constexpr int dbg_skip = 0;
#endif
    static const bool r2d_env_off = knob("H2AGG_REDUCE") && !strcmp(knob("H2AGG_REDUCE"), "segments");
    const int r2d_lc = p.NB == (uint32_t)(R2D_ROWS * R2D<7>::COLS) ? 7 : p.NB == (uint32_t)(R2D_ROWS * R2D<8>::COLS) ? 8 : 0;
    const bool r2d = !r2d_env_off && !c->cfg_seg && !pre && r2d_lc != 0;
    uint32_t* ticket = nullptr;
    if (r2d || fbdm) {
        DevBuf& tk = c->r2d_ticket[par];
        const size_t tickets = fbdm ? (size_t)FB_R2D_WINDOWS : (size_t)WT;
        if (tickets * 4 > tk.cap) {
            TRY(ensure(c, tk, tickets * 4));
            HIP_TRY(c, hipMemset(tk.p, 0, tk.cap));
        }
        ticket = (uint32_t*)tk.p;
    }
    debug_sync(4);
    const bool tails_off_stream = c->tail_overlap && c->overlap_level >= 2 && !split;
    const bool final_off_stream = c->tail_overlap && !split;
    uint8_t* const res_xyzz = c->d_res_xyzz;
    if (tails_off_stream) HIP_TRY(c, hipEventRecord(c->ev_bulk[par], st));
    auto tail_fn = [=](bool behind_sort) -> int {
        hipStream_t ts = st;
        if (tails_off_stream) {
// ... 490 lines not shown
    hipLaunchKernelGGL(k_g1_batch_to_affine, dim3(grid_for(c, n)), dim3(BLOCK), 0, c->stream, d_in_jac, n,
                       (uint8_t*)c->out.p, c->d_flags);
    HIP_TRY(c, hipMemcpyAsync(out, c->out.p, 64 * n, hipMemcpyDeviceToHost, c->stream));
    return finish(c);
} catch (const std::bad_alloc&) {
    return H2AGG_ERR_NOMEM;
} catch (...) {
    return H2AGG_ERR_INVALID;
}

int h2agg_g1_batch_decompress(h2agg_ctx* c, const uint8_t* in, size_t n, uint8_t* out_aff, uint8_t* ok) try {
    TRY(bind(c));
    if (n == 0) return H2AGG_OK;
    if (!in || !out_aff) return fail(c, H2AGG_ERR_INVALID, "null buffer");
    TRY(ensure(c, c->in_a, 32 * n));
    TRY(ensure(c, c->out, 64 * n));
    TRY(ensure(c, c->in_b, n + 16));
    HIP_TRY(c, hipMemcpyAsync(c->in_a.p, in, 32 * n, hipMemcpyHostToDevice, c->stream));
    TRY(clear_flags(c));
    hipLaunchKernelGGL(k_g1_batch_decompress, dim3(grid_for(c, n)), dim3(BLOCK), 0, c->stream, (const uint8_t*)c->in_a.p, n,
                       (uint8_t*)c->out.p, (uint8_t*)c->in_b.p, c->d_flags);
    HIP_TRY(c, hipMemcpyAsync(out_aff, c->out.p, 64 * n, hipMemcpyDeviceToHost, c->stream));
    if (ok) HIP_TRY(c, hipMemcpyAsync(ok, c->in_b.p, n, hipMemcpyDeviceToHost, c->stream));
    return finish(c);
} catch (const std::bad_alloc&) {
    return H2AGG_ERR_NOMEM;
} catch (...) {
    return H2AGG_ERR_INVALID;
}
int h2agg_g1_batch_compress(h2agg_ctx* c, const uint8_t* aff, size_t n, uint8_t* out) try {
    TRY(bind(c));
    if (n == 0) return H2AGG_OK;
    if (!aff || !out) return fail(c, H2AGG_ERR_INVALID, "null buffer");
    TRY(ensure(c, c->in_a, 64 * n));
    TRY(ensure(c, c->out, 32 * n));
    HIP_TRY(c, hipMemcpyAsync(c->in_a.p, aff, 64 * n, hipMemcpyHostToDevice, c->stream));
    TRY(clear_flags(c));
    hipLaunchKernelGGL(k_g1_batch_compress, dim3(grid_for(c, n)), dim3(BLOCK), 0, c->stream, (const uint8_t*)c->in_a.p, n,
                       (uint8_t*)c->out.p, c->d_flags);
    HIP_TRY(c, hipMemcpyAsync(out, c->out.p, 32 * n, hipMemcpyDeviceToHost, c->stream));
    return finish(c);
} catch (const std::bad_alloc&) {
    return H2AGG_ERR_NOMEM;
} catch (...) {
    return H2AGG_ERR_INVALID;
}

int h2agg_g1_sum(h2agg_ctx* c, const uint8_t* in, size_t n, uint8_t out[96]) try {
    TRY(bind(c));
    if (!out || (n && !in)) return fail(c, H2AGG_ERR_INVALID, "null buffer");
    TRY(ensure(c, c->in_a, 96 * n + 96));
    if (n) HIP_TRY(c, hipMemcpyAsync(c->in_a.p, in, 96 * n, hipMemcpyHostToDevice, c->stream));
    TRY(clear_flags(c));
    hipLaunchKernelGGL(k_g1_sum, dim3(1), dim3(BLOCK), 0, c->stream, (const uint8_t*)c->in_a.p, n, c->d_res_jac,
                       c->d_flags);
    return fetch_result_jac(c, out);
} catch (const std::bad_alloc&) {
    return H2AGG_ERR_NOMEM;
} catch (...) {
    return H2AGG_ERR_INVALID;
}

int h2agg_bases_upload(h2agg_ctx* c, const uint8_t* bases, size_t n, uint64_t* handle_out) try {
    TRY(bind(c));
    if (!bases || !handle_out || n == 0) return fail(c, H2AGG_ERR_INVALID, "null buffer or n == 0");
    Table t;
    t.n = n;
    if (hipMalloc((void**)&t.d, 64 * n) != hipSuccess) return fail(c, H2AGG_ERR_NOMEM, "hipMalloc(base table)");
    int rc = ensure(c, c->tmp_bases, 64 * n);
    if (rc == H2AGG_OK) {
        hipError_t e = hipMemcpyAsync(c->tmp_bases.p, bases, 64 * n, hipMemcpyHostToDevice, c->stream);
        if (e != hipSuccess) rc = fail(c, H2AGG_ERR_HIP, hipGetErrorString(e));
    }
    if (rc == H2AGG_OK) rc = clear_flags(c);
    if (rc == H2AGG_OK) {
        hipLaunchKernelGGL(k_bases_to_mont, dim3(grid_for(c, n)), dim3(BLOCK), 0, c->stream,
                           (const uint8_t*)c->tmp_bases.p, n, t.d, c->d_flags);
        rc = finish(c);
    }
    if (rc != H2AGG_OK) {
        hipFree(t.d);
        return rc;
    }
    uint64_t h = c->next_handle++;
    c->tables[h] = t;
    *handle_out = h;
    return H2AGG_OK;
} catch (const std::bad_alloc&) {
    return H2AGG_ERR_NOMEM;
} catch (...) {
    return H2AGG_ERR_INVALID;
}

}
namespace {
int comb_generate_launch(h2agg_ctx* c, const uint8_t* d_k, size_t n, uint8_t* out) {
    if (!c->comb_ready) {
        TRY(ensure(c, c->comb, (size_t)COMB_WINDOWS * COMB_ROW * 64));
        hipLaunchKernelGGL(k_comb_table_build, dim3((COMB_WINDOWS * COMB_ROW + SM_GROUPS - 1) / SM_GROUPS), dim3(SM_THREADS), 0,
                           c->stream, (uint8_t*)c->comb.p, c->d_flags);
        c->comb_ready = true;
    }
    size_t blocks = (n + BLOCK - 1) / BLOCK;
    if (blocks > 65535 * 16) blocks = 65535 * 16;
    hipLaunchKernelGGL(k_bases_generate_comb, dim3((unsigned)blocks), dim3(BLOCK), 0, c->stream, d_k, n, (const uint8_t*)c->comb.p,
                       out, c->d_flags);
    return H2AGG_OK;
}
}
extern "C" {
int h2agg_bases_generate(h2agg_ctx* c, const void* d_k, size_t n, uint64_t* handle_out) try {
    TRY(bind(c));
    if (!d_k || !handle_out || n == 0) return fail(c, H2AGG_ERR_INVALID, "null buffer or n == 0");
    Table t;
    t.n = n;
    if (hipMalloc((void**)&t.d, 64 * n) != hipSuccess) return fail(c, H2AGG_ERR_NOMEM, "hipMalloc(base table)");
    int rc = clear_flags(c);
    if (rc == H2AGG_OK) {
        static const bool ladder = knob("H2AGG_SCALAR_MUL") && !strcmp(knob("H2AGG_SCALAR_MUL"), "ladder");
        if (ladder) {
            size_t blocks = (n + BLOCK - 1) / BLOCK;
            if (blocks > 65535 * 16) blocks = 65535 * 16;
            hipLaunchKernelGGL(k_bases_generate, dim3((unsigned)blocks), dim3(BLOCK), 0, c->stream, (const uint8_t*)d_k, n, t.d,
                               c->d_flags);
        } else {
            rc = comb_generate_launch(c, (const uint8_t*)d_k, n, t.d);
        }
        if (rc == H2AGG_OK) rc = finish(c);
    }
    if (rc != H2AGG_OK) {
        hipFree(t.d);
        return rc;
    }
    uint64_t h = c->next_handle++;
    c->tables[h] = t;
    *handle_out = h;
    return H2AGG_OK;
} catch (const std::bad_alloc&) {
    return H2AGG_ERR_NOMEM;
} catch (...) {
    return H2AGG_ERR_INVALID;
}

int h2agg_bases_download(h2agg_ctx* c, uint64_t handle, size_t first, size_t n, uint8_t* out) try {
    TRY(bind(c));
    auto it = c->tables.find(handle);
    if (it == c->tables.end()) return fail(c, H2AGG_ERR_INVALID, "unknown base-table handle");
    if (!out || first + n > it->second.n) return fail(c, H2AGG_ERR_INVALID, "range outside the table");
    if (n == 0) return H2AGG_OK;
    TRY(ensure(c, c->out, 64 * n));
    hipLaunchKernelGGL(k_bases_from_mont, dim3(grid_for(c, n)), dim3(BLOCK), 0, c->stream, it->second.d + 64 * first,
                       n, (uint8_t*)c->out.p);
    HIP_TRY(c, hipMemcpyAsync(out, c->out.p, 64 * n, hipMemcpyDeviceToHost, c->stream));
    HIP_TRY(c, hipStreamSynchronize(c->stream));
    return H2AGG_OK;
} catch (const std::bad_alloc&) {
    return H2AGG_ERR_NOMEM;
} catch (...) {
    return H2AGG_ERR_INVALID;
}

int h2agg_bases_free(h2agg_ctx* c, uint64_t handle) try {
    TRY(bind(c));
    auto it = c->tables.find(handle);
    if (it == c->tables.end()) return fail(c, H2AGG_ERR_INVALID, "unknown base-table handle");
    TRY(join_tails(c));
    HIP_TRY(c, hipStreamSynchronize(c->stream));
    hipFree(it->second.d);
    if (it->second.endo_x) hipFree(it->second.endo_x);
    if (it->second.pre) hipFree(it->second.pre);
    it->second.free_combs();
    c->tables.erase(it);
    return H2AGG_OK;
} catch (const std::bad_alloc&) {
    return H2AGG_ERR_NOMEM;
} catch (...) {
    return H2AGG_ERR_INVALID;
}

}
namespace {
int table_endo(h2agg_ctx* c, Table& t, const uint8_t** out) {
    if (!t.endo_x) {
        if (hipMalloc((void**)&t.endo_x, 32 * t.n) != hipSuccess) return fail(c, H2AGG_ERR_NOMEM, "hipMalloc(endo table)");
        hipLaunchKernelGGL(k_bases_endo_x, dim3(grid_for(c, t.n)), dim3(BLOCK), 0, c->stream, (const uint8_t*)t.d, t.n,
                           t.endo_x);
    }
    *out = t.endo_x;
    return H2AGG_OK;
}
}
extern "C" {
int choose_pre_window(size_t n) {
    int best = 16;
    double best_cost = 1e300;
    for (int cc = 8; cc <= 20; ++cc) {
        const double cost = (double)n * ((255 + cc - 1) / cc) + 4.0 * (double)((size_t)1 << (cc - 1));
        if (cost < best_cost) {
            best_cost = cost;
            best = cc;
        }
    }
    return best;
}

int h2agg_bases_precompute(h2agg_ctx* c, uint64_t handle, int window_bits) try {
    TRY(bind(c));
    auto it = c->tables.find(handle);
    if (it == c->tables.end()) return fail(c, H2AGG_ERR_INVALID, "unknown base-table handle");
    Table& t = it->second;
    if (window_bits != 0 && (window_bits < 4 || window_bits > 20))
        return fail(c, H2AGG_ERR_INVALID, "fixed-base window must be 0 (auto) or in [4, 20]");
    int cc = window_bits ? window_bits : choose_pre_window(t.n);
    if (!window_bits && (size_t)((255 + cc - 1) / cc) * t.n > ((size_t)1 << 22)) cc = FB_C;
    const int W = (255 + cc - 1) / cc;
    if (cc == FB_C && t.n > (size_t)FB_MAX_TILES * FB_T)
// ... 6 lines not shown
        if ((size_t)W * t.n * 64 > free_b / 4)
            return fail(c, H2AGG_ERR_NOMEM, "fixed-base levels (auto) would take more than a quarter of the free device memory; pass window_bits to insist");
    }
    TRY(join_tails(c));
    HIP_TRY(c, hipStreamSynchronize(c->stream));
    if (t.pre) {
        hipFree(t.pre);
        t.pre = nullptr;
    }
    t.free_combs();
    if (hipMalloc((void**)&t.pre, (size_t)W * t.n * 64) != hipSuccess)
        return fail(c, H2AGG_ERR_NOMEM, "hipMalloc(fixed-base levels)");
    HIP_TRY(c, hipMemcpyAsync(t.pre, t.d, t.n * 64, hipMemcpyDeviceToDevice, c->stream));
    for (int w = 1; w < W; ++w)
        hipLaunchKernelGGL(k_bases_shift, dim3(grid_for(c, t.n)), dim3(BLOCK), 0, c->stream,
                           (const uint8_t*)t.pre + (size_t)(w - 1) * t.n * 64, t.n, cc, t.pre + (size_t)w * t.n * 64);
    HIP_TRY(c, hipStreamSynchronize(c->stream));
    t.pre_c = cc;
    t.pre_W = W;
    return H2AGG_OK;
} catch (const std::bad_alloc&) {
    return H2AGG_ERR_NOMEM;
} catch (...) {
    return H2AGG_ERR_INVALID;
}

}
namespace {
bool comb_msm_applies(const h2agg_ctx* c, const Table& t, size_t n) {
    const bool off = !c->dbg_comb_msm;
    return !off && t.pre && !c->cfg_c && n >= 1 && n <= (size_t)COMB_MSM_MAX;
}
int comb_msm_run(h2agg_ctx* c, Table& t, const uint8_t* d_scalars, size_t n, size_t batch, uint8_t* d_out_jac, bool* done) {
    *done = true;
    if (!t.comb || t.comb_n < n) {
        const size_t cap_n = t.n < (size_t)COMB_MSM_MAX ? t.n : (size_t)COMB_MSM_MAX;
        size_t nb = 16;
        while (nb < n) nb *= 2;
        if (nb > cap_n) nb = cap_n;
        const size_t entries = nb * (size_t)COMB_WINDOWS * COMB_ROW;
        uint8_t* fresh = nullptr;
        if (hipMalloc((void**)&fresh, entries * 64) != hipSuccess) {
            (void)hipGetLastError();
            *done = false;
            return H2AGG_OK;
        }
        if (t.comb) t.comb_retired.push_back(t.comb);
        t.comb = fresh;
        size_t grid = (entries + SM_GROUPS - 1) / SM_GROUPS;
        const size_t cap = (size_t)c->cu_count * 16;
        if (grid > cap) grid = cap;
        hipLaunchKernelGGL(k_comb_table_build, dim3((unsigned)grid), dim3(SM_THREADS), 0, c->stream, t.comb, c->d_flags,
                           (const uint8_t*)t.d, (uint32_t)nb);
        t.comb_n = nb;
    }
    hipLaunchKernelGGL(k_comb_msm, dim3((unsigned)batch), dim3(BLOCK), 0, c->stream, (const uint8_t*)t.comb, d_scalars, (uint32_t)n,
                       d_out_jac, c->d_flags);
    HIP_TRY(c, hipGetLastError());
    return H2AGG_OK;
}
}
extern "C" {

int h2agg_g1_msm_device_async(h2agg_ctx* c, uint64_t handle, const void* d_scalars, size_t n, void* d_out_jac) try {
    TRY(bind(c));
    auto it = c->tables.find(handle);
    if (it == c->tables.end()) return fail(c, H2AGG_ERR_INVALID, "unknown base-table handle");
    if (!d_scalars || !d_out_jac) return fail(c, H2AGG_ERR_INVALID, "null buffer");
    if (n == 0) return fail(c, H2AGG_ERR_EMPTY, "multi_exp of zero pairs (reference panics: mock/arith/ecc.rs:128)");
    if (n > it->second.n) return fail(c, H2AGG_ERR_INVALID, "more scalars than bases in the table");
    if (comb_msm_applies(c, it->second, n)) {
        bool done = false;
        TRY(comb_msm_run(c, it->second, (const uint8_t*)d_scalars, n, 1, (uint8_t*)d_out_jac, &done));
        if (done) return H2AGG_OK;
    }
    const uint8_t* endo = nullptr;
    TRY(table_endo(c, it->second, &endo));
    if (it->second.pre && !c->cfg_c) {
        const PreTable pt{it->second.pre, it->second.n, it->second.pre_c, it->second.pre_W};
        if ((size_t)pt.W * n < ((size_t)1 << 32))
            return msm_run(c, it->second.d, (const uint8_t*)d_scalars, n, (uint8_t*)d_out_jac, 1, nullptr, &pt);
    }
    const size_t SLICE = (size_t)1 << 22;
    if (n <= SLICE) return msm_run(c, it->second.d, (const uint8_t*)d_scalars, n, (uint8_t*)d_out_jac, 1, endo);
    const size_t nsl = (n + SLICE - 1) / SLICE;
    const bool was_overlap = c->tail_overlap;
    const int was_level = c->overlap_level;
    c->tail_overlap = true;
    c->overlap_level = 2;
    c->chain_n = n;
    c->chain_glv = false;
    int rc = H2AGG_OK;
    for (size_t k = 0; k < nsl && rc == H2AGG_OK; ++k) {
        const size_t off = k * SLICE, m = n - off < SLICE ? n - off : SLICE;
        c->chain = k == 0 ? CHAIN_FIRST : (k + 1 == nsl ? CHAIN_LAST : CHAIN_MID);
        rc = msm_run(c, it->second.d + 64 * off, (const uint8_t*)d_scalars + 32 * off, m, (uint8_t*)d_out_jac, 1, endo + 32 * off);
    }
    c->chain = CHAIN_OFF;
    c->tail_overlap = was_overlap;
    c->overlap_level = was_level;
    TRY(rc);
    if (!was_overlap) TRY(join_tails(c));
    return H2AGG_OK;
} catch (const std::bad_alloc&) {
    return H2AGG_ERR_NOMEM;
} catch (...) {
    return H2AGG_ERR_INVALID;
}

int h2agg_g1_msm_device_batch_async(h2agg_ctx* c, uint64_t handle, const void* d_scalars, size_t n, size_t batch,
                                    void* d_out_jac) try {
    TRY(bind(c));
    auto it = c->tables.find(handle);
    if (it == c->tables.end()) return fail(c, H2AGG_ERR_INVALID, "unknown base-table handle");
    if (!d_scalars || !d_out_jac) return fail(c, H2AGG_ERR_INVALID, "null buffer");
    if (n == 0 || batch == 0)
        return fail(c, H2AGG_ERR_EMPTY, "multi_exp of zero pairs (reference panics: mock/arith/ecc.rs:128)");
    if (n > it->second.n) return fail(c, H2AGG_ERR_INVALID, "more scalars than bases in the table");
    if (comb_msm_applies(c, it->second, n)) {
        bool done = false;
        TRY(comb_msm_run(c, it->second, (const uint8_t*)d_scalars, n, batch, (uint8_t*)d_out_jac, &done));
        if (done) return H2AGG_OK;
    }
    const bool fb_table = it->second.pre && it->second.pre_c == FB_C && !c->dbg_pre_big;
    const bool use_pre = it->second.pre && !c->cfg_c && (!fb_table || (fb_sort_knobs_clear(c) && (batch == 1 || n >= ((size_t)1 << 18))));
    const PreTable pt{it->second.pre, it->second.n, it->second.pre_c, it->second.pre_W};
    const MsmPlan p1 = make_plan(c, n, 1);
    const uint32_t nb1 = use_pre ? (1u << (pt.c - 1)) : p1.NB;
    const size_t sets1 = use_pre ? 1 : (size_t)p1.W;
    uint32_t ppw_min = nb1 >> 11;
    if (ppw_min < 1) ppw_min = 1;
    size_t per = (size_t)SORT_MAX_PW / (sets1 * ppw_min);
    const size_t ent1 = use_pre ? n * (size_t)pt.W : n * (size_t)p1.W * (p1.glv ? 2 : 1);
    if (per * ent1 >= ((size_t)1 << 31)) per = (((size_t)1 << 31) - 1) / ent1;
    if (per * n >= ((size_t)1 << 29)) per = (((size_t)1 << 29) - 1) / n;
    if (per < 1) per = 1;
    const bool one_by_one = use_pre ? (pt.c == FB_C && n >= ((size_t)1 << 18)) : n >= ((size_t)1 << 20);
    if (one_by_one) per = 1;
    const uint8_t* endo = nullptr;
    TRY(table_endo(c, it->second, &endo));
    const bool was_overlap = c->tail_overlap;
    const int was_level = c->overlap_level;
    if (one_by_one && batch > 1) {
        c->tail_overlap = true;
        c->overlap_level = 2;
    }
    int rc = H2AGG_OK;
    for (size_t q = 0; q < batch && rc == H2AGG_OK; q += per) {
        const size_t b = batch - q < per ? batch - q : per;
        rc = msm_run(c, it->second.d, (const uint8_t*)d_scalars + 32 * n * q, n, (uint8_t*)d_out_jac + 96 * q, (uint32_t)b,
                     use_pre ? nullptr : endo, use_pre ? &pt : nullptr);
    }
    c->tail_overlap = was_overlap;
    c->overlap_level = was_level;
    TRY(rc);
    if (one_by_one && batch > 1 && !was_overlap) TRY(join_tails(c));
    return H2AGG_OK;
} catch (const std::bad_alloc&) {
    return H2AGG_ERR_NOMEM;
} catch (...) {
    return H2AGG_ERR_INVALID;
}

int h2agg_g1_msm_device(h2agg_ctx* c, uint64_t handle, const void* d_scalars, size_t n, uint8_t out[96]) try {
    TRY(bind(c));
    if (!out) return fail(c, H2AGG_ERR_INVALID, "null buffer");
    set_identity_jac(out);
    TRY(clear_flags(c));
    TRY(h2agg_g1_msm_device_async(c, handle, d_scalars, n, c->d_res_jac));
    return fetch_result_jac(c, out);
} catch (const std::bad_alloc&) {
    return H2AGG_ERR_NOMEM;
} catch (...) {
    return H2AGG_ERR_INVALID;
}

int h2agg_g1_msm_preloaded(h2agg_ctx* c, uint64_t handle, const uint8_t* scalars, size_t n, uint8_t out[96]) try {
    TRY(bind(c));
    if (!out) return fail(c, H2AGG_ERR_INVALID, "null buffer");
    set_identity_jac(out);
    if (n == 0) return fail(c, H2AGG_ERR_EMPTY, "multi_exp of zero pairs (reference panics: mock/arith/ecc.rs:128)");
    if (!scalars) return fail(c, H2AGG_ERR_INVALID, "null buffer");
    TRY(ensure(c, c->in_b, 32 * n));
    HIP_TRY(c, hipMemcpyAsync(c->in_b.p, scalars, 32 * n, hipMemcpyHostToDevice, c->stream));
    return h2agg_g1_msm_device(c, handle, c->in_b.p, n, out);
} catch (const std::bad_alloc&) {
    return H2AGG_ERR_NOMEM;
} catch (...) {
    return H2AGG_ERR_INVALID;
}

int h2agg_instance_commitment(h2agg_ctx* c, uint64_t g_lagrange_handle, const uint8_t* instance, size_t len,
                              size_t max_len, uint8_t out_jac[96]) try {
    TRY(bind(c));
    if (!out_jac) return fail(c, H2AGG_ERR_INVALID, "null buffer");
    set_identity_jac(out_jac);
    if (len > max_len)
        return fail(c, H2AGG_ERR_INVALID, "assert!(instance.len() <= params.n() - (blinding_factors + 1)) failed (verify.rs:601-603)");
    if (len == 0) return H2AGG_OK;
    return h2agg_g1_msm_preloaded(c, g_lagrange_handle, instance, len, out_jac);
} catch (const std::bad_alloc&) {
    return H2AGG_ERR_NOMEM;
} catch (...) {
    return H2AGG_ERR_INVALID;
}

int h2agg_host_alloc(h2agg_ctx* c, size_t bytes, void** out) try {
    TRY(bind(c));
    if (!out || bytes == 0) return fail(c, H2AGG_ERR_INVALID, "null out or zero size");
    hipError_t e = hipHostMalloc(out, bytes, hipHostMallocDefault);
    if (e != hipSuccess) return fail(c, H2AGG_ERR_NOMEM, std::string("hipHostMalloc: ") + hipGetErrorString(e));
    return H2AGG_OK;
} catch (const std::bad_alloc&) {
    return H2AGG_ERR_NOMEM;
} catch (...) {
    return H2AGG_ERR_INVALID;
}
int h2agg_host_free(h2agg_ctx* c, void* p) try {
    TRY(bind(c));
    if (p) HIP_TRY(c, hipHostFree(p));
    return H2AGG_OK;
} catch (const std::bad_alloc&) {
    return H2AGG_ERR_NOMEM;
} catch (...) {
    return H2AGG_ERR_INVALID;
}

}
namespace {
int msm_host(h2agg_ctx* c, const uint8_t* bases, size_t stride, const uint8_t* scalars, size_t n, uint8_t out[96]);
}
extern "C" {
int h2agg_g1_msm(h2agg_ctx* c, const uint8_t* bases, const uint8_t* scalars, size_t n, uint8_t out[96]) try {
    return msm_host(c, bases, 64, scalars, n, out);
// ... 166 lines not shown
    if (mode < -1 || mode > 1) return fail(c, H2AGG_ERR_INVALID, "mode must be -1 (off), 0 (auto) or 1 (on)");
    c->cfg_glv = mode;
    return H2AGG_OK;
} catch (const std::bad_alloc&) {
    return H2AGG_ERR_NOMEM;
} catch (...) {
    return H2AGG_ERR_INVALID;
}
int h2agg_msm_configure_lanes_per_bucket(h2agg_ctx* c, int lanes) try {
    if (!c) return H2AGG_ERR_INVALID;
    if (lanes != 0 && lanes != 1 && lanes != 2 && lanes != 4 && lanes != 8 && lanes != 16)
        return fail(c, H2AGG_ERR_INVALID, "lanes must be 0, 1, 2, 4, 8 or 16");
    c->cfg_lpb = lanes;
    return H2AGG_OK;
} catch (const std::bad_alloc&) {
    return H2AGG_ERR_NOMEM;
} catch (...) {
    return H2AGG_ERR_INVALID;
}

int h2agg_msm_configure_sort(h2agg_ctx* c, int sub_bits, int tile) try {
    if (!c) return H2AGG_ERR_INVALID;
    if (sub_bits != 0 && (sub_bits < 4 || sub_bits > SORT_MAX_SUB_BITS))
        return fail(c, H2AGG_ERR_INVALID, "sub_bits must be 0 or in [4, 12]");
    if (tile != 0 && tile != -1 && tile != -2 && tile != -3 && (tile < BLOCK || tile > (1 << 16)))
        return fail(c, H2AGG_ERR_INVALID, "tile must be 0, -1, -2 or in [256, 65536]");
    c->cfg_sub_bits = sub_bits;
    c->cfg_no_stage = tile == -1;
    c->cfg_no_dm = tile == -3;
    c->cfg_stage_l1 = tile == -2;
    c->cfg_tile = tile > 0 ? tile : 0;
    return H2AGG_OK;
} catch (const std::bad_alloc&) {
    return H2AGG_ERR_NOMEM;
} catch (...) {
    return H2AGG_ERR_INVALID;
}

int h2agg_debug_configure(h2agg_ctx* c, const char* key, int value) try {
    if (!c || !key) return H2AGG_ERR_INVALID;
    const std::string k(key);
    if (k == "pcie_slices") c->dbg_pcie_slices = value;
    else if (k == "pcie_glv") c->dbg_pcie_glv = value;
    else if (k == "pcie_chain") c->dbg_pcie_chain = value;
    else if (k == "comb_msm") c->dbg_comb_msm = value;
    else if (k == "plan_cache") c->dbg_plan_cache = value;
    else if (k == "small_sort") c->dbg_small_sort = value;
    else if (k == "eval_split") c->dbg_eval_split = value;
    else if (k == "shard_fail") c->dbg_shard_fail = value;
    else if (k == "lean_acc") {
#ifdef H2AGG_MEASURE_KNOBS
        c->dbg_lean_acc = value;
#else
        if (value != 1) return fail(c, H2AGG_ERR_INVALID, "h2agg_debug_configure: the generic accumulation kernel is in the measure build only (build_ext.py --measure)");
#endif
    }
    else if (k == "tape_lds") {
        if (c->dbg_tape_lds != value) agg_plans_release(c);
        c->dbg_tape_lds = value;
    }
    else if (k == "prewake") c->dbg_prewake = value;
    else if (k == "phases") c->dbg_phases = value;
    else if (k == "seg_chunk") c->dbg_seg_chunk = value;
    else if (k == "seg_c") {
        if (value != 0 && (value < 4 || value > 8)) return fail(c, H2AGG_ERR_INVALID, "h2agg_debug_configure: seg_c must be 0 or 4 .. 8");
        c->dbg_seg_c = value;
    }
    else if (k == "fr_fft_local") {
        if (value < 0 || value > (int)FR_FFT_TILE_LOG) return fail(c, H2AGG_ERR_INVALID, "h2agg_debug_configure: fr_fft_local must be 0 or 1 .. 11");
        c->dbg_fr_fft_local = value;
    }
    else if (k == "fr_poly_chunk") {
        if (value != 0 && (value < (int)FR_CHUNK_PER_LOG || value > (int)FR_CHUNK_LOG)) return fail(c, H2AGG_ERR_INVALID, "h2agg_debug_configure: fr_poly_chunk must be 0 or 3 .. 11");
        c->dbg_fr_poly_chunk = value;
    }
    else if (k == "fr_scan_chunk") {
        if (value != 0 && (value < (int)FR_CHUNK_PER_LOG || value > (int)FR_CHUNK_LOG)) return fail(c, H2AGG_ERR_INVALID, "h2agg_debug_configure: fr_scan_chunk must be 0 or 3 .. 11");
        c->dbg_fr_scan_chunk = value;
    }
    else if (k == "fr_sort_tile") {
        if (value != 0 && (value < (int)LK_TILE_LOG_MIN || value > (int)LK_TILE_LOG)) return fail(c, H2AGG_ERR_INVALID, "h2agg_debug_configure: fr_sort_tile must be 0 or 4 .. 11");
        c->dbg_fr_sort_tile = value;
    }
    else if (k == "pre_big") c->dbg_pre_big = value;
    else return fail(c, H2AGG_ERR_INVALID, "h2agg_debug_configure: unknown key " + k);
    return H2AGG_OK;
} catch (...) {
    return H2AGG_ERR_INVALID;
}

int h2agg_msm_set_tail_overlap(h2agg_ctx* c, int enable) try {
    TRY(bind(c));
    TRY(join_tails(c));
    HIP_TRY(c, hipStreamSynchronize(c->stream));
    c->tail_overlap = enable != 0;
    if (enable >= 1 && enable <= 3) c->overlap_level = enable;
    return H2AGG_OK;
} catch (const std::bad_alloc&) {
    return H2AGG_ERR_NOMEM;
} catch (...) {
    return H2AGG_ERR_INVALID;
}

int h2agg_profile_enable(h2agg_ctx* c, int enable) try {
    TRY(bind(c));
    if (enable && !c->prof_events_created) {
        for (int r = 0; r < h2agg_ctx::PROF_RING; ++r)
            for (int s = 0; s < ST_N; ++s)
                for (int k = 0; k < 2; ++k) HIP_TRY(c, hipEventCreateWithFlags(&c->prof[r].ev[s][k], EV_TIME_FLAGS));
        c->prof_events_created = true;
    }
    if (!enable) profile_harvest_all(c);
    c->profiling = enable != 0;
    c->prof_only = (enable >= 2 && enable - 2 < ST_N) ? enable - 2 : -1;
    return H2AGG_OK;
} catch (const std::bad_alloc&) {
    return H2AGG_ERR_NOMEM;
} catch (...) {
    return H2AGG_ERR_INVALID;
}
int h2agg_profile_reset(h2agg_ctx* c) try {
    if (!c) return H2AGG_ERR_INVALID;
    profile_harvest_all(c);
    for (int s = 0; s < ST_N; ++s) {
        c->stage_ms[s] = 0;
        c->stage_launches[s] = 0;
    }
    return H2AGG_OK;
} catch (const std::bad_alloc&) {
    return H2AGG_ERR_NOMEM;
} catch (...) {
    return H2AGG_ERR_INVALID;
}
int h2agg_profile_stage_count(h2agg_ctx*) { return ST_N; }
const char* h2agg_profile_stage_name(h2agg_ctx*, int i) { return (i >= 0 && i < ST_N) ? STAGE_NAMES[i] : ""; }
int h2agg_profile_stage_get(h2agg_ctx* c, int i, double* total_ms, uint64_t* launches) try {
    if (!c || i < 0 || i >= ST_N) return H2AGG_ERR_INVALID;
    profile_harvest_all(c);
    if (total_ms) *total_ms = c->stage_ms[i];
    if (launches) *launches = c->stage_launches[i];
    return H2AGG_OK;
} catch (const std::bad_alloc&) {
    return H2AGG_ERR_NOMEM;
} catch (...) {
    return H2AGG_ERR_INVALID;
}

extern "C++" {
namespace {
bool host_pool_pair_if_awake(const std::function<void()>& on_worker, const std::function<void()>& here);
bool pairing_adx_ok() {
#ifdef H2AGG_PAIRING_ADX_BUILD
    static const bool ok = __builtin_cpu_supports("bmi2") && __builtin_cpu_supports("adx") && !getenv("H2AGG_PAIRING_PORTABLE");
    return ok;
#else
    return false;
#endif
}
template <class P>
int pairing_load(h2agg_ctx* c, const uint8_t* g1_aff, const uint8_t* g2_aff, size_t n, std::vector<typename P::G1>& ps,
                 std::vector<typename P::G2>& qs) {
    if (n && (!g1_aff || !g2_aff)) return fail(c, H2AGG_ERR_INVALID, "null buffer");
    ps.resize(n);
    qs.resize(n);
    for (size_t i = 0; i < n; ++i) {
        const int r1 = P::load1(g1_aff + 64 * i, ps[i]);
        if (r1 == 1) return fail(c, H2AGG_ERR_NONCANONICAL, "pairing: G1 coordinate >= p");
        if (r1) return fail(c, H2AGG_ERR_BAD_POINT, "pairing: G1 point not on the curve");
// ... 123 lines not shown
```

### halo2-snark-aggregator_amd/csrc/msm_kernels.hpp

```cpp
#pragma once
#include "sort_kernels.hpp"
#include "fb_sort_kernels.hpp"

namespace h2agg {

struct MsmPlan {
    int c;
    int W;
    uint32_t NB;
    uint32_t NBT;
    uint32_t seg;
    uint32_t spw;
    uint32_t big;
    bool glv;
};

FP_INLINE G1Affine msm_gather(const uint8_t* __restrict__ bases, const uint8_t* __restrict__ endo_x, uint32_t e) {
    const size_t idx = e & ENT_IDX;
    G1Affine p;
    p.x = fp_load<FqParams>((e & ENT_ENDO) ? endo_x + 32 * idx : bases + 64 * idx);
    p.y = fp_load<FqParams>(bases + 64 * idx + 32);
    return (e & ENT_NEG) ? affine_neg(p) : p;
}
__global__ void __launch_bounds__(BLOCK) k_bases_endo_x(const uint8_t* __restrict__ bases, size_t n,
// ... 24 lines not shown
    cs = cs < BIG_CHUNK ? BIG_CHUNK : (cs > BIG_CHUNK_MAX ? BIG_CHUNK_MAX : cs);
    return cs;
}

template <int CHAIN>
__global__ void __launch_bounds__(BLOCK) k_msm_accumulate(const uint8_t* __restrict__ bases,
                                                          const uint8_t* __restrict__ endo_x,
                                                          const uint32_t* __restrict__ entries,
                                                          const uint32_t* __restrict__ offs,
                                                          const uint32_t* __restrict__ hist,
                                                          const uint32_t* __restrict__ order, uint32_t nbt, uint32_t big,
                                                          uint32_t lpb ,
                                                          uint8_t* __restrict__ buckets, uint32_t* __restrict__ big_list,
                                                          uint32_t* __restrict__ big_keys,
                                                          uint32_t* __restrict__ counters ) {
    const uint32_t t = blockIdx.x * blockDim.x + threadIdx.x;
    if (t >= nbt * lpb) return;
    const uint32_t part = t % lpb;
    const uint32_t key = order ? order[t / lpb] : t / lpb;
    const uint32_t len = hist[key];
    if (len > big) {
        if (part != 0) {
            if (CHAIN == 1) xyzz_store(buckets + XYZZ_BYTES * ((size_t)key * lpb + part), G1XYZZ::identity());
            return;
        }
        const uint32_t cs = big_chunk_size(len);
        const uint32_t nch = (len + cs - 1) / cs;
        const uint32_t base = atomicAdd(&counters[0], nch);
        for (uint32_t j = 0; j < nch; ++j) {
            big_list[3 * (base + j)] = key;
            big_list[3 * (base + j) + 1] = j;
            big_list[3 * (base + j) + 2] = nch;
        }
        if (nch > 1) {
            const uint32_t k = atomicAdd(&counters[1], 1u);
            big_keys[3 * k] = key;
            big_keys[3 * k + 1] = base;
            big_keys[3 * k + 2] = nch;
        }
        return;
    }
    const uint32_t lo = (uint32_t)(((uint64_t)len * part) / lpb), hi = (uint32_t)(((uint64_t)len * (part + 1)) / lpb);
    const uint32_t* run = entries + offs[key];
    G1XYZZ acc = G1XYZZ::identity();
    uint32_t k0 = lo;
    bool fresh = true;
    if (CHAIN == 2) {
        if (hi == lo) return;
        acc = xyzz_load(buckets + XYZZ_BYTES * ((size_t)key * lpb + part));
        fresh = acc.is_identity();
    }
    G1Affine first;
    bool have_first = false;
    while (fresh && k0 < hi && !have_first) {
        first = msm_gather(bases, endo_x, run[k0++]);
        have_first = !first.is_identity();
    }
    G1Affine second;
    bool have_second = false;
    while (have_first && k0 < hi && !have_second) {
        second = msm_gather(bases, endo_x, run[k0++]);
        have_second = !second.is_identity();
    }
    if (have_second) acc = xyzz_add_affine_affine(first, second);
    else if (have_first) acc = G1XYZZ::from_affine(first);
    if (hi > k0) {
        const uint32_t lo = k0;
        G1Affine nxt = msm_gather(bases, endo_x, run[lo]);
        uint32_t e_after = lo + 1 < hi ? run[lo + 1] : 0u;
#pragma unroll 1
        for (uint32_t k = lo; k < hi; ++k) {
            G1Affine cur = nxt;
            if (k + 1 < hi) {
                nxt = msm_gather(bases, endo_x, e_after);
                e_after = k + 2 < hi ? run[k + 2] : 0u;
            }
            xyzz_add_affine(acc, cur);
        }
    }
    xyzz_store(buckets + XYZZ_BYTES * ((size_t)key * lpb + part), acc);
}

struct RawPt { uint4 a, b, c, d; };
FP_INLINE RawPt raw_gather(const uint8_t* __restrict__ bases, const uint8_t* __restrict__ endo_x, uint32_t e) {
    const size_t idx = e & ENT_IDX;
    const uint4* px = reinterpret_cast<const uint4*>((e & ENT_ENDO) ? endo_x + 32 * idx : bases + 64 * idx);
    const uint4* py = reinterpret_cast<const uint4*>(bases + 64 * idx + 32);
    RawPt r;
    r.a = px[0]; r.b = px[1]; r.c = py[0]; r.d = py[1];
    return r;
}
FP_INLINE G1Affine raw_unpack(const RawPt& r, uint32_t e) {
    G1Affine p;
    { uint32_t w[8] = {r.a.x, r.a.y, r.a.z, r.a.w, r.b.x, r.b.y, r.b.z, r.b.w}; p.x = fp_unpack<FqParams>(w); }
    { uint32_t w[8] = {r.c.x, r.c.y, r.c.z, r.c.w, r.d.x, r.d.y, r.d.z, r.d.w}; p.y = fp_unpack<FqParams>(w); }
    return (e & ENT_NEG) ? affine_neg(p) : p;
}
template <bool DUAL, class NextF>
FP_INLINE bool xyzz_add_affine_lean(G1XYZZ& acc, G1Affine q, NextF&& issue_next) {
    bool ok = !q.is_identity() && !acc.is_identity();
    if (DUAL) {
        fpa_mul_dual_ip<FqParams>(q.x, acc.zz, q.y, acc.zzz);
    } else {
        fpa_mul_ip<FqParams>(q.x, acc.zz);
        fpa_mul_ip<FqParams>(q.y, acc.zzz);
    }
    Fq p = FQ_SUB(8, q.x, acc.x);
    Fq r = FQ_SUB(4, q.y, acc.y);
    ok = ok && !fp_maybe_zero_mod2<10, FqParams>(p);
    if (!ok) return false;
    Fq pp, rr;
    if (DUAL) {
        fpa_sqr_dual<FqParams>(pp, rr, p, r);
        fpa_mul_dual_ip<FqParams>(p, pp, acc.x, pp);
    } else {
        fpa_sqr<FqParams>(pp, p);
        fpa_sqr<FqParams>(rr, r);
        fpa_mul_ip<FqParams>(p, pp);
        fpa_mul_ip<FqParams>(acc.x, pp);
    }
    Fq x3 = fp_sub_sub2<6, FqParams>(rr, p, acc.x);
    Fq d = FQ_SUB(8, acc.x, x3);
    acc.x = x3;
    Fq ny = fp_neg<4, FqParams>(acc.y);
    if (DUAL) {
        fpa_mul_dual_ip<FqParams>(acc.zz, pp, acc.zzz, p);
        issue_next();
        fpa_mul2_ip<FqParams>(ny, p, r, d);
    } else {
        fpa_mul_ip<FqParams>(acc.zz, pp);
        fpa_mul_ip<FqParams>(acc.zzz, p);
        fpa_mul2_ip1<FqParams>(ny, p, r, d);
    }
    acc.y = ny;
    return true;
}
template <bool DUAL>
FP_INLINE bool xyzz_add_affine_affine_lean(G1XYZZ& o, const G1Affine& a, const G1Affine& q) {
    Fq p = FQ_SUB(2, q.x, a.x);
    Fq r = FQ_SUB(2, q.y, a.y);
    if (q.is_identity() || fp_maybe_zero_mod2<4, FqParams>(p)) return false;
    Fq pp, rr;
    Fq qq = a.x;
    if (DUAL) {
        fpa_sqr_dual<FqParams>(pp, rr, p, r);
        fpa_mul_dual_ip<FqParams>(p, pp, qq, pp);
    } else {
        fpa_sqr<FqParams>(pp, p);
        fpa_sqr<FqParams>(rr, r);
        fpa_mul_ip<FqParams>(p, pp);
        fpa_mul_ip<FqParams>(qq, pp);
    }
    o.x = fp_sub_sub2<6, FqParams>(rr, p, qq);
    Fq d = FQ_SUB(8, qq, o.x);
    Fq ny = fp_neg<2, FqParams>(a.y);
    if (DUAL) fpa_mul2_ip<FqParams>(ny, p, r, d);
    else fpa_mul2_ip1<FqParams>(ny, p, r, d);
    o.y = ny;
    o.zz = pp;
    o.zzz = p;
    return true;
}

template <int CHAIN, bool DUAL>
__global__ void __launch_bounds__(64) __attribute__((amdgpu_waves_per_eu(4, 4)))
k_msm_accumulate_lean(const uint8_t* __restrict__ bases, const uint8_t* __restrict__ endo_x,
                      const uint32_t* __restrict__ entries, const uint32_t* __restrict__ offs,
                      const uint32_t* __restrict__ hist, const uint32_t* __restrict__ order, uint32_t nbt, uint32_t big,
                      uint32_t lpb, uint8_t* __restrict__ buckets, uint32_t* __restrict__ big_list,
                      uint32_t* __restrict__ big_keys, uint32_t* __restrict__ counters, uint32_t* __restrict__ fix_list) {
    const uint32_t t = blockIdx.x * blockDim.x + threadIdx.x;
    if (t >= nbt * lpb) return;
    const uint32_t part = t % lpb;
    const uint32_t key = order ? order[t / lpb] : t / lpb;
    const uint32_t len = hist[key];
    const uint32_t slot = key * lpb + part;
    if (len > big) {
        if (part != 0) {
            if (CHAIN == 1) xyzz_store(buckets + XYZZ_BYTES * (size_t)slot, G1XYZZ::identity());
            return;
        }
        const uint32_t cs = big_chunk_size(len);
        const uint32_t nch = (len + cs - 1) / cs;
        const uint32_t base = atomicAdd(&counters[0], nch);
        for (uint32_t j = 0; j < nch; ++j) {
            big_list[3 * (base + j)] = key;
            big_list[3 * (base + j) + 1] = j;
            big_list[3 * (base + j) + 2] = nch;
        }
        if (nch > 1) {
            const uint32_t kk = atomicAdd(&counters[1], 1u);
            big_keys[3 * kk] = key;
            big_keys[3 * kk + 1] = base;
            big_keys[3 * kk + 2] = nch;
        }
        return;
    }
    const uint32_t lo = (uint32_t)(((uint64_t)len * part) / lpb), hi = (uint32_t)(((uint64_t)len * (part + 1)) / lpb);
    const uint32_t roff = offs[key];
    auto run = [&](uint32_t i) { return entries[roff + i]; };
    G1XYZZ acc = G1XYZZ::identity();
    if (CHAIN == 2) {
        if (hi == lo) return;
        acc = xyzz_load(buckets + XYZZ_BYTES * (size_t)slot);
    }
    uint32_t k = lo;
    if (hi > lo) {
        uint32_t e_cur = run(lo);
        RawPt nxt = raw_gather(bases, endo_x, e_cur);
        uint32_t e_nxt = run(lo + 1 < hi ? lo + 1 : hi - 1);
        auto advance = [&](uint32_t k_now) {
            e_cur = e_nxt;
            nxt = raw_gather(bases, endo_x, e_nxt);
            e_nxt = run(k_now + 2 < hi ? k_now + 2 : hi - 1);
        };
        bool go = true;
        if (acc.is_identity()) {
            const G1Affine first = raw_unpack(nxt, e_cur);
            go = !first.is_identity();
            if (go) {
                advance(lo);
                k = lo + 1;
                acc = G1XYZZ::from_affine(first);
                if (k < hi) {
                    const G1Affine second = raw_unpack(nxt, e_cur);
                    advance(lo + 1);
                    go = xyzz_add_affine_affine_lean<DUAL>(acc, first, second);
                    if (go) k = lo + 2;
                }
            }
        }
        if (go) {
#pragma unroll 1
            for (; k < hi; ++k) {
                const G1Affine cur = raw_unpack(nxt, e_cur);
                if (!xyzz_add_affine_lean<DUAL>(acc, cur, [&]() { advance(k); })) break;
            }
        }
        if (k < hi) {
            const uint32_t f = atomicAdd(&counters[2], 1u);
            fix_list[2 * f] = slot;
            fix_list[2 * f + 1] = k;
        }
    }
    uint32_t oslot = slot;
    asm volatile("" : "+v"(oslot));
    xyzz_store(buckets + XYZZ_BYTES * (size_t)oslot, acc);
}
__global__ void __launch_bounds__(64) k_msm_accumulate_fix(const uint8_t* __restrict__ bases, const uint8_t* __restrict__ endo_x,
                                                           const uint32_t* __restrict__ entries,
                                                           const uint32_t* __restrict__ offs,
                                                           const uint32_t* __restrict__ hist, uint32_t lpb,
                                                           uint8_t* __restrict__ buckets,
                                                           const uint32_t* __restrict__ counters,
                                                           const uint32_t* __restrict__ fix_list) {
    const uint32_t nfix = counters[2];
    for (uint32_t f = blockIdx.x * 64 + threadIdx.x; f < nfix; f += gridDim.x * 64) {
        const uint32_t slot = fix_list[2 * f], k0 = fix_list[2 * f + 1];
        const uint32_t key = slot / lpb, part = slot - key * lpb;
        const uint32_t len = hist[key];
        const uint32_t hi = (uint32_t)(((uint64_t)len * (part + 1)) / lpb);
        const uint32_t* run = entries + offs[key];
        G1XYZZ acc = xyzz_load(buckets + XYZZ_BYTES * (size_t)slot);
#pragma unroll 1
        for (uint32_t k = k0; k < hi; ++k) xyzz_add_affine(acc, msm_gather(bases, endo_x, run[k]));
        xyzz_store(buckets + XYZZ_BYTES * (size_t)slot, acc);
    }
}

__global__ void __launch_bounds__(BLOCK) k_msm_bucket_combine(const uint8_t* __restrict__ parts,
                                                              const uint32_t* __restrict__ hist, uint32_t nbt,
                                                              uint32_t big, uint32_t lpb, uint8_t* __restrict__ buckets) {
    const uint32_t key = blockIdx.x * BLOCK + threadIdx.x;
    if (key >= nbt) return;
    G1XYZZ acc = xyzz_load(parts + XYZZ_BYTES * (size_t)key * lpb);
    if (hist[key] <= big) {
#pragma unroll 1
        for (uint32_t j = 1; j < lpb; ++j) acc = xyzz_add(acc, xyzz_load(parts + XYZZ_BYTES * ((size_t)key * lpb + j)));
    }
    xyzz_store(buckets + XYZZ_BYTES * (size_t)key, acc);
}

__device__ __noinline__ G1XYZZ wave_sum_xyzz(G1XYZZ v, uint32_t* lds) {
    const int lane = threadIdx.x;
    auto put = [&](int slot, const G1XYZZ& p) {
#pragma unroll
        for (int i = 0; i < NL; ++i) {
            lds[i * 64 + slot] = p.x.l[i];
            lds[(NL + i) * 64 + slot] = p.y.l[i];
            lds[(2 * NL + i) * 64 + slot] = p.zz.l[i];
            lds[(3 * NL + i) * 64 + slot] = p.zzz.l[i];
        }
    };
    put(lane, v);
    __syncthreads();
#pragma unroll 1
    for (int s2 = 32; s2 >= 1; s2 >>= 1) {
        if (lane < s2) {
            G1XYZZ o;
#pragma unroll
            for (int i = 0; i < NL; ++i) {
                o.x.l[i] = lds[i * 64 + lane + s2];
                o.y.l[i] = lds[(NL + i) * 64 + lane + s2];
                o.zz.l[i] = lds[(2 * NL + i) * 64 + lane + s2];
                o.zzz.l[i] = lds[(3 * NL + i) * 64 + lane + s2];
            }
            v = xyzz_add(v, o);
            put(lane, v);
        }
        __syncthreads();
    }
    return v;
}

__global__ void __launch_bounds__(64) k_msm_accumulate_big(const uint8_t* __restrict__ bases,
                                                           const uint8_t* __restrict__ endo_x,
                                                           const uint32_t* __restrict__ entries,
                                                           const uint32_t* __restrict__ offs,
                                                           const uint32_t* __restrict__ hist,
                                                           uint8_t* __restrict__ buckets, uint32_t stride ,
                                                           uint8_t* __restrict__ big_part,
                                                           const uint32_t* __restrict__ big_list,
                                                           const uint32_t* __restrict__ counters,
                                                           uint32_t resume ) {
    __shared__ uint32_t lds[XYZZ_WORDS * 64];
    const uint32_t nslots = counters[0];
    for (uint32_t b = blockIdx.x; b < nslots; b += gridDim.x) {
        const uint32_t key = big_list[3 * b], chunk = big_list[3 * b + 1], nch = big_list[3 * b + 2];
        const uint32_t len = hist[key];
        const uint32_t cs = big_chunk_size(len);
        const uint32_t lo = chunk * cs, hi = (lo + cs < len) ? lo + cs : len;
// ... 528 lines not shown
```

### halo2-snark-aggregator_amd/csrc/params.inc

```

namespace {

struct DevTmp {
    void* p = nullptr;
    ~DevTmp() {
        if (p) hipFree(p);
    }
    int alloc(h2agg_ctx* c, size_t bytes, const char* what) {
        if (hipMalloc(&p, bytes ? bytes : 1) != hipSuccess) {
            p = nullptr;
            return fail(c, H2AGG_ERR_NOMEM, std::string("hipMalloc(") + what + ")");
        }
        return H2AGG_OK;
    }
};

constexpr size_t FRP_CST_BYTES = 32 * (FRP_TABLE + 2);

int fr_affine_powers_launch(h2agg_ctx* c, ph::HFr base, const ph::HFr& A, const ph::HFr& B, size_t n, uint8_t* d_cst, uint8_t* d_out) {
    uint8_t cst[FRP_CST_BYTES];
    for (int j = 0; j < FRP_TABLE; ++j) {
        hfr_bytes(base, cst + 32 * j);
        base = ph::mul(base, base);
    }
// ... 39 lines not shown
    HIP_TRY(c, hipMemcpy(d.p, sc, sizeof sc, hipMemcpyHostToDevice));
    hipLaunchKernelGGL(k_fft_twiddle_digits, dim3(1), dim3(BLOCK), 0, c->stream, (const uint8_t*)d.p, cnt, (uint32_t*)c->fft_scale.p,
                       c->d_flags);
    HIP_TRY(c, hipStreamSynchronize(c->stream));
    c->fft_scale_ready = true;
    return H2AGG_OK;
}

int fft_run(h2agg_ctx* c, const uint8_t* d_in, unsigned k, int inv, uint8_t* d_out) {
    const size_t n = (size_t)1 << k;
    DevTmp work, jac;
    TRY(work.alloc(c, XYZZ_BYTES * n, "FFT work array"));
    TRY(jac.alloc(c, 96 * n, "FFT result"));
    TRY(clear_flags(c));
    if (k) TRY(fft_ensure_twiddles(c, k, inv));
    const uint32_t* scale = nullptr;
    if (k && inv) {
        TRY(fft_ensure_scale(c));
        scale = (const uint32_t*)c->fft_scale.p + (size_t)FFT_REC_WORDS * k;
    }
    hipStream_t st = c->stream;
    hipLaunchKernelGGL(k_g1_fft_load, dim3((unsigned)((n + SM_GROUPS - 1) / SM_GROUPS)), dim3(SM_THREADS), 0, st, d_in, (uint32_t)k,
                       scale, (uint8_t*)work.p);
    const unsigned grid = (unsigned)((n / 2 + SM_GROUPS - 1) / SM_GROUPS);
    const uint32_t* tw = (const uint32_t*)c->fft_tw[inv].p;
    const uint32_t tw_shift = k ? (uint32_t)(c->fft_tw_k[inv] - (int)k) : 0u;
    for (unsigned s = 1; s <= k; ++s) {
        if (((uint32_t)1 << (k - s)) >= FFT_UNIFORM_MIN)
            hipLaunchKernelGGL(k_g1_fft_stage<true>, dim3(grid), dim3(SM_THREADS), 0, st, (uint8_t*)work.p, (uint32_t)k, (uint32_t)s, tw,
                               tw_shift);
        else
            hipLaunchKernelGGL(k_g1_fft_stage<false>, dim3(grid), dim3(SM_THREADS), 0, st, (uint8_t*)work.p, (uint32_t)k, (uint32_t)s, tw,
                               tw_shift);
    }
    hipLaunchKernelGGL(k_g1_fft_to_jac, dim3(grid_for(c, n)), dim3(BLOCK), 0, st, (const uint8_t*)work.p, n, (uint8_t*)jac.p);
    hipLaunchKernelGGL(k_jac_to_mont_affine, dim3(grid_for(c, n)), dim3(BLOCK), 0, st, (const uint8_t*)jac.p, n, d_out, c->d_flags);
    HIP_TRY(c, hipGetLastError());
    return finish(c);
}

int params_setup_run(h2agg_ctx* c, unsigned k, const ph::HFr& s, const ph::HFr& s_n, uint8_t* d_g, uint8_t* d_gl) {
    const size_t n = (size_t)1 << k;
    DevTmp scal, invs, cst;
    TRY(scal.alloc(c, 32 * n, "setup scalars"));
    TRY(cst.alloc(c, 2 * FRP_CST_BYTES, "setup constants"));
    if (d_gl) TRY(invs.alloc(c, 32 * n, "setup scalars"));
    TRY(clear_flags(c));
    if (d_g) {
        TRY(fr_affine_powers_launch(c, s, ph::one(), ph::zero(), n, (uint8_t*)cst.p, (uint8_t*)scal.p));
        TRY(comb_generate_launch(c, (const uint8_t*)scal.p, n, d_g));
    }
    if (d_gl) {
        const ph::HFr cinv = ph::inv(ph::mul(ph::sub(s_n, ph::one()), ph::inv(hfr_u64((uint64_t)n))));
        TRY(fr_affine_powers_launch(c, ph::inv(fft_omega(k)), ph::mul(s, cinv), ph::sub(ph::zero(), cinv), n,
                                    (uint8_t*)cst.p + FRP_CST_BYTES, (uint8_t*)scal.p));
        hipLaunchKernelGGL(k_fr_batch_op, dim3(grid_for(c, n)), dim3(BLOCK), 0, c->stream, (int)H2AGG_OP_INV, (const uint8_t*)scal.p,
                           (const uint8_t*)nullptr, n, (uint8_t*)invs.p, c->d_flags);
        TRY(comb_generate_launch(c, (const uint8_t*)invs.p, n, d_gl));
    }
    HIP_TRY(c, hipGetLastError());
    return finish(c);
}

}

extern "C" {

int h2agg_bases_fft(h2agg_ctx* c, uint64_t in_handle, unsigned k, int inverse, uint64_t* out_handle) try {
    TRY(bind(c));
    if (!out_handle) return fail(c, H2AGG_ERR_INVALID, "null handle pointer");
    if (k > FFT_MAX_K) return fail(c, H2AGG_ERR_INVALID, "k must be <= 24");
    auto it = c->tables.find(in_handle);
    if (it == c->tables.end()) return fail(c, H2AGG_ERR_INVALID, "unknown base-table handle");
    const size_t n = (size_t)1 << k;
    if (n > it->second.n) return fail(c, H2AGG_ERR_INVALID, "the table has fewer than 2^k points");
    Table t;
    t.n = n;
    if (hipMalloc((void**)&t.d, 64 * n) != hipSuccess) return fail(c, H2AGG_ERR_NOMEM, "hipMalloc(base table)");
    const int rc = fft_run(c, it->second.d, k, inverse ? 1 : 0, t.d);
    if (rc != H2AGG_OK) {
        hipFree(t.d);
        return rc;
    }
    const uint64_t h = c->next_handle++;
    c->tables[h] = t;
    *out_handle = h;
    return H2AGG_OK;
} catch (const std::bad_alloc&) {
    return H2AGG_ERR_NOMEM;
} catch (...) {
    return H2AGG_ERR_INVALID;
}

int h2agg_params_setup(h2agg_ctx* c, unsigned k, const uint8_t s[32], uint64_t* g_handle_out, uint64_t* g_lagrange_handle_out) try {
    TRY(bind(c));
    if (!s) return fail(c, H2AGG_ERR_INVALID, "null buffer");
    if (k > FFT_MAX_K) return fail(c, H2AGG_ERR_INVALID, "k must be <= 24");
    if (!fr_bytes_canonical(s)) return fail(c, H2AGG_ERR_NONCANONICAL, "input integer >= modulus");
    uint64_t sw[4];
    memcpy(sw, s, 32);
    const ph::HFr sm = ph::from_words(sw);
    if (ph::is_zero(sm)) return fail(c, H2AGG_ERR_INVALID, "setup: s == 0 (every g[i], i > 0, would be the identity)");
    ph::HFr s_n = sm;
    for (unsigned i = 0; i < k; ++i) s_n = ph::mul(s_n, s_n);
    if (ph::is_zero(ph::sub(s_n, ph::one())))
        return fail(c, H2AGG_ERR_INVALID, "setup: s^n == 1 (halo2: (s - w^i).invert().unwrap() panics)");
    const size_t n = (size_t)1 << k;
    Table tg, tl;
    tg.n = tl.n = n;
    if (g_handle_out && hipMalloc((void**)&tg.d, 64 * n) != hipSuccess) return fail(c, H2AGG_ERR_NOMEM, "hipMalloc(base table)");
    if (g_lagrange_handle_out && hipMalloc((void**)&tl.d, 64 * n) != hipSuccess) {
        if (tg.d) hipFree(tg.d);
        return fail(c, H2AGG_ERR_NOMEM, "hipMalloc(base table)");
    }
    const int rc = (tg.d || tl.d) ? params_setup_run(c, k, sm, s_n, tg.d, tl.d) : H2AGG_OK;
    if (rc != H2AGG_OK) {
        if (tg.d) hipFree(tg.d);
        if (tl.d) hipFree(tl.d);
        return rc;
    }
    if (tg.d) {
        const uint64_t h = c->next_handle++;
        c->tables[h] = tg;
        *g_handle_out = h;
    }
    if (tl.d) {
        const uint64_t h = c->next_handle++;
        c->tables[h] = tl;
        *g_lagrange_handle_out = h;
    }
    return H2AGG_OK;
} catch (const std::bad_alloc&) {
    return H2AGG_ERR_NOMEM;
} catch (...) {
    return H2AGG_ERR_INVALID;
}

int h2agg_g2_scalar_mul(const uint8_t g2_aff[128], const uint8_t s[32], uint8_t out_aff[128]) try {
    if (!g2_aff || !s || !out_aff) return H2AGG_ERR_INVALID;
    pairing::G2Affine q;
    const int r = pairing::load_g2(g2_aff, q);
    if (r == 1) return H2AGG_ERR_NONCANONICAL;
    if (r) return H2AGG_ERR_BAD_POINT;
    if (!fr_bytes_canonical(s)) return H2AGG_ERR_NONCANONICAL;
    uint64_t e[4];
    memcpy(e, s, 32);
    int top = 255;
    while (top >= 0 && !((e[top / 64] >> (top % 64)) & 1)) --top;
    if (top < 0 || q.inf) {
        memset(out_aff, 0, 128);
        return H2AGG_OK;
    }
    pairing::G2Proj acc = {q.x, q.y, pairing::f2_one()};
    for (int i = top - 1; i >= 0; --i) {
        pairing::g2_double_step(acc);
        if ((e[i / 64] >> (i % 64)) & 1) pairing::g2_add_step(acc, q);
    }
    const pairing::Fq2 zi = pairing::f2_inv(acc.z);
    const pairing::G2Affine o = {pairing::f2_mul(acc.x, zi), pairing::f2_mul(acc.y, zi), false};
    pairing::g2_to_bytes(o, out_aff);
    return H2AGG_OK;
} catch (const std::bad_alloc&) {
    return H2AGG_ERR_NOMEM;
} catch (...) {
    return H2AGG_ERR_INVALID;
}

int h2agg_g2_batch_compress(const uint8_t* aff, size_t n, uint8_t* out) try {
    if (n && (!aff || !out)) return H2AGG_ERR_INVALID;
    for (size_t i = 0; i < n; ++i) {
        const uint8_t* b = aff + 128 * i;
        pairing::G2Affine q;
        bool zero = true;
        for (int j = 0; j < 128; ++j) zero &= b[j] == 0;
        q.inf = zero;
        if (!pairing::fq_from_bytes(b, q.x.c0) || !pairing::fq_from_bytes(b + 32, q.x.c1) || !pairing::fq_from_bytes(b + 64, q.y.c0) ||
            !pairing::fq_from_bytes(b + 96, q.y.c1))
            return H2AGG_ERR_NONCANONICAL;
        if (!pairing::g2_on_curve(q)) return H2AGG_ERR_BAD_POINT;
        memcpy(out + 64 * i, b, 64);
        if (!zero) out[64 * i + 63] |= (uint8_t)((b[64] & 1) << 7);
    }
    return H2AGG_OK;
} catch (const std::bad_alloc&) {
    return H2AGG_ERR_NOMEM;
} catch (...) {
    return H2AGG_ERR_INVALID;
}

}
```

### halo2-snark-aggregator_amd/csrc/scalar_mul_kernels.hpp

```cpp
#pragma once
#include "msm_kernels.hpp"

namespace h2agg {

constexpr int SM_THREADS = 128;
constexpr int SM_GROUPS = SM_THREADS / 4;
constexpr int SM_TABLE = 8;

struct W4Digits {
    uint32_t mag[5];
    uint64_t neg;
};
FP_INLINE W4Digits w4_recode(const uint32_t (&m)[4]) {
    W4Digits r;
#pragma unroll
    for (int i = 0; i < 5; ++i) r.mag[i] = 0;
    r.neg = 0;
    uint32_t carry = 0;
#pragma unroll
    for (int j = 0; j < 33; ++j) {
        const uint32_t nib = (j < 32 ? ((m[j >> 3] >> (4 * (j & 7))) & 15u) : 0u) + carry;
        const bool ng = nib > 8u;
        carry = ng ? 1u : 0u;
        const uint32_t mg = ng ? 16u - nib : nib;
// ... 73 lines not shown
            acc = xyzz_add_par4(acc, q);
        }
    }
    return acc;
}

__global__ void __launch_bounds__(SM_THREADS) k_g1_batch_scalar_mul_w4(const uint8_t* __restrict__ bases,
                                                                        const uint8_t* __restrict__ scalars, size_t n,
                                                                        uint8_t* __restrict__ out, uint32_t* flags) {
    __shared__ uint32_t tab[SM_TABLE * XYZZ_WORDS * SM_GROUPS];
    const size_t ngroups_total = (size_t)gridDim.x * SM_GROUPS;
    for (size_t i0 = (size_t)blockIdx.x * SM_GROUPS; i0 < n; i0 += ngroups_total) {
        const size_t i = i0 + (threadIdx.x >> 2);
        const bool live = i < n;
        const size_t ii = live ? i : n - 1;
        uint32_t bad = 0;
        const G1Affine p = affine_load_canonical(bases + 64 * ii, bad);
        const U256 s = u256_load(scalars + 32 * ii);
        bad |= !u256_is_canonical_fr(s);
        if (bad && live) atomicOr(flags, FLAG_NONCANONICAL);
        G1XYZZ r = G1XYZZ::identity();
        if (!p.is_identity()) r = g1_scalar_mul_w4_par4(p, s, tab, flags);
        if (live && (threadIdx.x & 3) == 0) jac_store_canonical(out + 96 * i, jac_from_xyzz(r));
        __syncthreads();
    }
}

constexpr int COMB_BITS = 8, COMB_WINDOWS = 32, COMB_ROW = (1 << COMB_BITS) - 1;

__global__ void __launch_bounds__(SM_THREADS) k_comb_table_build(uint8_t* __restrict__ table, uint32_t* flags,
                                                                 const uint8_t* __restrict__ bases = nullptr, uint32_t nb = 1) {
    __shared__ uint32_t tab[SM_TABLE * XYZZ_WORDS * SM_GROUPS];
    const size_t per_base = (size_t)COMB_WINDOWS * COMB_ROW;
    const size_t total = per_base * nb;
    const size_t ngroups_total = (size_t)gridDim.x * SM_GROUPS;
    for (size_t e0 = (size_t)blockIdx.x * SM_GROUPS; e0 < total; e0 += ngroups_total) {
        const size_t e = e0 + (threadIdx.x >> 2);
        const bool live = e < total;
        const size_t ee = live ? e : total - 1;
        const size_t bi = ee / per_base, er = ee - bi * per_base;
        const uint32_t w = (uint32_t)(er / COMB_ROW), dgt = (uint32_t)(er % COMB_ROW) + 1u;
        U256 s;
#pragma unroll
        for (int k = 0; k < 8; ++k) s.w[k] = 0;
        s.w[w >> 2] = dgt << (8 * (w & 3));
#pragma unroll 1
        for (int it = 0; it < 6; ++it) {
            if (u256_is_canonical_fr(s)) break;
            uint64_t br = 0;
            const uint32_t rw[8] = {0xf0000001u, 0x43e1f593u, 0x79b97091u, 0x2833e848u, 0x8181585du, 0xb85045b6u, 0xe131a029u, 0x30644e72u};
#pragma unroll
            for (int k = 0; k < 8; ++k) {
                const uint64_t dd = (uint64_t)s.w[k] - rw[k] - br;
                s.w[k] = (uint32_t)dd;
                br = (dd >> 32) & 1;
            }
        }
        G1Affine gen;
        if (bases) {
            gen = affine_load(bases + 64 * bi);
        } else {
            gen.x = Fq::one();
            gen.y = FQ_DBL(Fq::one());
        }
        G1XYZZ r = G1XYZZ::identity();
        if (!gen.is_identity()) r = g1_scalar_mul_w4_par4(gen, s, tab, flags);
        if (live && (threadIdx.x & 3) == 0) affine_store(table + 64 * e, affine_from_xyzz(r));
        __syncthreads();
    }
}

__global__ void __launch_bounds__(BLOCK) k_bases_generate_comb(const uint8_t* __restrict__ k, size_t n,
                                                               const uint8_t* __restrict__ table,
                                                               uint8_t* __restrict__ out, uint32_t* flags) {
    for (size_t i = (size_t)blockIdx.x * BLOCK + threadIdx.x; i < n; i += (size_t)gridDim.x * BLOCK) {
        const U256 s = u256_load(k + 32 * i);
        if (!u256_is_canonical_fr(s)) atomicOr(flags, FLAG_NONCANONICAL);
        G1XYZZ acc = G1XYZZ::identity();
#pragma unroll 1
        for (int w = 0; w < COMB_WINDOWS; ++w) {
            const uint32_t d = (s.w[w >> 2] >> (8 * (w & 3))) & 0xffu;
            if (d) xyzz_add_affine(acc, affine_load(table + 64 * ((size_t)w * COMB_ROW + d - 1)));
        }
        affine_store(out + 64 * i, affine_from_xyzz(acc));
    }
}

constexpr int COMB_MSM_MAX = 256;
__global__ void __launch_bounds__(BLOCK) k_comb_msm(const uint8_t* __restrict__ table, const uint8_t* __restrict__ scalars,
                                                    uint32_t n, uint8_t* __restrict__ out_jac, uint32_t* flags) {
    __shared__ uint32_t lds[XYZZ_WORDS * BLOCK];
    const uint8_t* sc = scalars + 32 * (size_t)n * blockIdx.x;
    G1XYZZ acc = G1XYZZ::identity();
    bool bad = false;
#pragma unroll 1
    for (uint32_t e = threadIdx.x; e < n * (uint32_t)COMB_WINDOWS; e += BLOCK) {
        const uint32_t i = e / COMB_WINDOWS, w = e % COMB_WINDOWS;
        if (w == 0) bad |= !u256_is_canonical_fr(u256_load(sc + 32 * (size_t)i));
        const uint32_t d = sc[32 * (size_t)i + w];
        if (d) xyzz_add_affine(acc, affine_load(table + 64 * (((size_t)i * COMB_WINDOWS + w) * COMB_ROW + d - 1)));
    }
    if (bad) atomicOr(flags, FLAG_NONCANONICAL);
    const G1XYZZ tot = block_sum_xyzz(acc, lds);
    if (threadIdx.x == 0) jac_store_canonical(out_jac + 96 * (size_t)blockIdx.x, jac_from_xyzz(tot));
}

}
```

### include/h2agg.h

```cpp
#ifndef H2AGG_H
#define H2AGG_H

#include <stddef.h>
#include <stdint.h>

#ifdef __cplusplus
extern "C" {
#endif

typedef struct h2agg_ctx h2agg_ctx;

enum {
    H2AGG_OK = 0,
    H2AGG_ERR_INVALID = 1,
    H2AGG_ERR_DIV_ZERO = 2,
    H2AGG_ERR_EMPTY = 3,
    H2AGG_ERR_HIP = 4,
    H2AGG_ERR_NONCANONICAL = 5,
    H2AGG_ERR_NOMEM = 6,
    H2AGG_ERR_BAD_POINT = 7,
    H2AGG_ERR_PEER = 8,
    H2AGG_ERR_NOT_IN_TABLE = 9
};

// ... 140 lines not shown
int h2agg_comm_unique_id(uint8_t out[128]);
int h2agg_comm_init_rank(h2agg_ctx* ctx, const uint8_t id[128], int rank, int nranks);
int h2agg_comm_create(const int* devices, int ndev, h2agg_ctx** ctxs_out);
int h2agg_comm_size(h2agg_ctx* ctx);
int h2agg_comm_rank(h2agg_ctx* ctx);
const char* h2agg_comm_last_error(void);
int h2agg_allgather_add_points(h2agg_ctx** ctxs, int nctx, const uint8_t* partial_jac, size_t npts, uint8_t* out_aff);

int h2agg_pairing_check(h2agg_ctx* ctx, const uint8_t* g1_aff, const uint8_t* g2_aff, size_t n, int* ok);
int h2agg_g2_batch_decompress(h2agg_ctx* ctx, const uint8_t* in, size_t n, uint8_t* out_aff);
int h2agg_pairing_product(h2agg_ctx* ctx, const uint8_t* g1_aff, const uint8_t* g2_aff, size_t n, uint8_t out_gt[384]);
int h2agg_final_pair_check(h2agg_ctx* ctx, const uint8_t left_aff[64], const uint8_t right_aff[64],
                           const uint8_t s_g2[128], const uint8_t g2[128], int* ok);

int h2agg_bases_fft(h2agg_ctx* ctx, uint64_t in_handle, unsigned k, int inverse, uint64_t* out_handle);

int h2agg_params_setup(h2agg_ctx* ctx, unsigned k, const uint8_t s[32], uint64_t* g_handle_out, uint64_t* g_lagrange_handle_out);

int h2agg_g2_scalar_mul(const uint8_t g2_aff[128], const uint8_t s[32], uint8_t out_aff[128]);
int h2agg_g2_batch_compress(const uint8_t* aff, size_t n, uint8_t* out);

int h2agg_fr_fft(h2agg_ctx* ctx, const uint8_t* in, unsigned k, int inverse, const uint8_t shift[32], uint8_t* out);
int h2agg_fr_fft_device(h2agg_ctx* ctx, const void* d_in, unsigned k, int inverse, const uint8_t shift[32], void* d_out);

int h2agg_fr_poly_eval(h2agg_ctx* ctx, const uint8_t* polys, size_t npoly, unsigned k, const uint32_t* queries, size_t nq,
                       const uint8_t* points, size_t npoints, uint8_t* out);
int h2agg_fr_poly_eval_device(h2agg_ctx* ctx, const void* d_polys, size_t npoly, unsigned k, const uint32_t* queries, size_t nq,
                              const uint8_t* points, size_t npoints, uint8_t* out);
int h2agg_fr_poly_divide(h2agg_ctx* ctx, const uint8_t* in, unsigned k, const uint8_t z[32], uint8_t* out, uint8_t rem[32]);
int h2agg_fr_poly_divide_device(h2agg_ctx* ctx, const void* d_poly, unsigned k, const uint8_t z[32], void* d_quot, void* d_rem);
int h2agg_kzg_multiopen(h2agg_ctx* ctx, uint64_t g_handle, const uint8_t* polys, size_t npoly, unsigned k, const uint32_t* queries,
                        size_t nq, const uint8_t* points, size_t npoints, const uint8_t v[32], uint8_t* w_aff,
                        uint32_t* group_points, size_t* ngroups);
int h2agg_kzg_multiopen_device(h2agg_ctx* ctx, uint64_t g_handle, const void* d_polys, size_t npoly, unsigned k,
                               const uint32_t* queries, size_t nq, const uint8_t* points, size_t npoints, const uint8_t v[32],
                               uint8_t* w_aff, uint32_t* group_points, size_t* ngroups);

int h2agg_fr_batch_invert(h2agg_ctx* ctx, const uint8_t* in, size_t n, uint8_t* out);
int h2agg_fr_batch_invert_device(h2agg_ctx* ctx, const void* d_in, size_t n, void* d_out);
int h2agg_fr_grand_product(h2agg_ctx* ctx, const uint8_t* num, const uint8_t* den, unsigned k, size_t u, const uint8_t init[32],
                           uint8_t* out, uint8_t last[32]);
int h2agg_fr_grand_product_device(h2agg_ctx* ctx, const void* d_num, const void* d_den, unsigned k, size_t u, const uint8_t init[32],
                                  void* d_out, void* d_last);
int h2agg_permutation_product(h2agg_ctx* ctx, const uint8_t* values, const uint8_t* sigmas, size_t m, unsigned k, size_t u,
                              const uint8_t beta[32], const uint8_t gamma[32], const uint8_t delta[32],
                              const uint8_t delta_first[32], const uint8_t init[32], uint8_t* out, uint8_t last[32]);
int h2agg_permutation_product_device(h2agg_ctx* ctx, const void* d_values, const void* d_sigmas, size_t m, unsigned k, size_t u,
                                     const uint8_t beta[32], const uint8_t gamma[32], const uint8_t delta[32],
                                     const uint8_t delta_first[32], const uint8_t init[32], void* d_out, void* d_last);
int h2agg_lookup_product(h2agg_ctx* ctx, const uint8_t* a, const uint8_t* s, const uint8_t* ap, const uint8_t* sp, unsigned k,
                         size_t u, const uint8_t beta[32], const uint8_t gamma[32], uint8_t* out, uint8_t last[32]);
int h2agg_lookup_product_device(h2agg_ctx* ctx, const void* d_a, const void* d_s, const void* d_ap, const void* d_sp, unsigned k,
                                size_t u, const uint8_t beta[32], const uint8_t gamma[32], void* d_out, void* d_last);

int h2agg_lookup_permute(h2agg_ctx* ctx, const uint8_t* a, const uint8_t* s, unsigned k, size_t u, uint8_t* ap, uint8_t* sp);
int h2agg_lookup_permute_device(h2agg_ctx* ctx, const void* d_a, const void* d_s, unsigned k, size_t u, void* d_ap, void* d_sp);
int h2agg_fr_columns_compress(h2agg_ctx* ctx, const uint8_t* cols, size_t m, unsigned k, const uint8_t theta[32], uint8_t* out);
int h2agg_fr_columns_compress_device(h2agg_ctx* ctx, const void* d_cols, size_t m, unsigned k, const uint8_t theta[32], void* d_out);

#define H2AGG_EXPR_MAX_DEPTH 16
int h2agg_vk_expressions_eval(h2agg_ctx* ctx, const h2agg_vk* vk, int which, size_t j, unsigned k, const uint8_t* advice,
                              const uint8_t* fixed, const uint8_t* instance, const uint8_t* challenges, const uint8_t fold[32],
                              uint8_t* out);
int h2agg_vk_expressions_eval_device(h2agg_ctx* ctx, const h2agg_vk* vk, int which, size_t j, unsigned k, const void* d_advice,
                                     const void* d_fixed, const void* d_instance, const uint8_t* challenges, const uint8_t fold[32],
                                     void* d_out);
int h2agg_quotient(h2agg_ctx* ctx, const h2agg_vk* vk, const uint8_t* advice, const uint8_t* fixed, const uint8_t* instance,
                   const uint8_t* sigma, const uint8_t* perm_z, const uint8_t* lookup_z, const uint8_t* lookup_ap,
                   const uint8_t* lookup_sp, const uint8_t* challenges, const uint8_t theta[32], const uint8_t beta[32],
                   const uint8_t gamma[32], const uint8_t y[32], const uint8_t delta[32], uint8_t* h);
int h2agg_quotient_device(h2agg_ctx* ctx, const h2agg_vk* vk, const void* d_advice, const void* d_fixed, const void* d_instance,
                          const void* d_sigma, const void* d_perm_z, const void* d_lookup_z, const void* d_lookup_ap,
                          const void* d_lookup_sp, const uint8_t* challenges, const uint8_t theta[32], const uint8_t beta[32],
                          const uint8_t gamma[32], const uint8_t y[32], const uint8_t delta[32], void* d_h);

int h2agg_fr_tape_eval(h2agg_ctx* ctx, const uint8_t* consts, size_t nconst, const uint32_t* ops3, size_t nops,
                       const uint32_t* out_regs, size_t nout, uint8_t* out);

int h2agg_msm_configure(h2agg_ctx* ctx, int window_bits, int reduce_segment, int big_bucket_threshold);
int h2agg_msm_configure_glv(h2agg_ctx* ctx, int mode);
int h2agg_msm_configure_lanes_per_bucket(h2agg_ctx* ctx, int lanes);
int h2agg_msm_configure_sort(h2agg_ctx* ctx, int sub_bits, int tile);
int h2agg_debug_configure(h2agg_ctx* ctx, const char* key, int value);
int h2agg_msm_set_tail_overlap(h2agg_ctx* ctx, int enable);
int h2agg_profile_enable(h2agg_ctx* ctx, int enable);
int h2agg_profile_reset(h2agg_ctx* ctx);
int h2agg_profile_stage_count(h2agg_ctx* ctx);
const char* h2agg_profile_stage_name(h2agg_ctx* ctx, int i);
int h2agg_profile_stage_get(h2agg_ctx* ctx, int i, double* total_ms, uint64_t* launches);

#ifdef __cplusplus
}
#endif
#endif
```

Baseline: 835.0 million.

## Specialize lean MSM accumulate on identity-free tables and GLV usage, fold sign into subtraction

Base-table upload kernels now raise a flag when any base is the identity, and each table records whether it is identity-free. The lean bucket-accumulate kernel gets template variants that drop the per-add identity check and the endomorphism x-select when they are not needed. Point negation is folded into the y subtraction through a sign mask instead of a separate affine_neg, and some subtractions skip normalization by using borrowed limb constants. The cost is more kernel instantiations and an atomic flag write during table load, and the loose limb bounds depend on the later multiplies accepting unnormalized inputs.

```diff
diff --git a/halo2-snark-aggregator_amd/__init__.py b/halo2-snark-aggregator_amd/__init__.py
--- a/halo2-snark-aggregator_amd/__init__.py
+++ b/halo2-snark-aggregator_amd/__init__.py
@@ -127,6 +127,8 @@
         "h2agg_verify_aggregation_ex": (i32, [ctxp, vp, sz, u8p, u8p, vp, vp, vp, C.POINTER(i32), vp, sz]),
         "h2agg_verify_aggregation_sharded": (i32, [ctxp, vp, sz, vp, u8p, u8p, vp, vp, vp, C.POINTER(i32), vp, sz]),
         "h2agg_debug_configure": (i32, [ctxp, C.c_char_p, i32]),
+        "h2agg_debug_lean_variant": (i32, [i32, i32]),
+        "h2agg_debug_table_identity": (i32, [ctxp, u64, C.POINTER(i32), C.POINTER(i32)]),
         "h2agg_verify_proofs": (i32, [ctxp, vp, sz, u8p, u8p, vp, vp, C.POINTER(C.c_int32), C.POINTER(i32), vp, sz]),
         "h2agg_verify_plan_stats": (i32, [ctxp, C.POINTER(C.c_uint64), C.POINTER(C.c_uint64), C.POINTER(C.c_uint64)]),
         "h2agg_last_phases": (C.c_char_p, [ctxp]),
@@ -841,6 +843,16 @@
     def debug_configure(self, key: str, value: int):
         self._check(self._lib.h2agg_debug_configure(self._ctx, key.encode(), int(value)))
 
+    def table_may_hold_identity(self, handle: int) -> bool:
+        v = C.c_int32(-1)
+        self._check(self._lib.h2agg_debug_table_identity(self._ctx, handle, C.byref(v), None))
+        return bool(v.value)
+
+    def last_lean_variant(self) -> int:
+        v = C.c_int32(-1)
+        self._check(self._lib.h2agg_debug_table_identity(self._ctx, 0, None, C.byref(v)))
+        return v.value
+
     def msm_set_tail_overlap(self, level: int = 2):
         self._check(self._lib.h2agg_msm_set_tail_overlap(self._ctx, int(level)))
 
diff --git a/halo2-snark-aggregator_amd/csrc/batch_kernels.hpp b/halo2-snark-aggregator_amd/csrc/batch_kernels.hpp
--- a/halo2-snark-aggregator_amd/csrc/batch_kernels.hpp
+++ b/halo2-snark-aggregator_amd/csrc/batch_kernels.hpp
@@ -10,7 +10,9 @@
 __global__ void k_flags_roll(uint32_t* flags) {
     flags[2] |= flags[0];
     flags[0] = 0;
-}
+    flags[1] = 0;
+}
+#define NOTE_IDENTITY_BASE(flags, is_id) do { if (is_id) atomicOr((flags) + 1, 1u); } while (0)
 
 template <int NLIMB>
 FP_INLINE void lds_put(uint32_t* lds, int tid, const uint32_t* v) {
@@ -301,6 +303,7 @@
                     oy = fp_from_mont<FqParams>(oy);
                 }
             }
+            if (MONT) NOTE_IDENTITY_BASE(flags, ox.is_zero_int() && oy.is_zero_int());
             fp_store<FqParams>(out + 64 * i, ox);
             fp_store<FqParams>(out + 64 * i + 32, oy);
         }
@@ -435,6 +438,7 @@
         uint32_t bad = 0;
         G1Affine p = affine_load_canonical(in + 64 * i, bad);
         if (bad) atomicOr(flags, FLAG_NONCANONICAL);
+        NOTE_IDENTITY_BASE(flags, p.is_identity());
         affine_store(out + 64 * i, p);
     }
 }
@@ -454,8 +458,10 @@
         G1Affine g;
         g.x = Fq::one();
         g.y = FQ_DBL(Fq::one());
-        affine_store(out + 64 * i, affine_from_xyzz(g1_scalar_mul(g, s)));
-    }
-}
-
-}
+        const G1Affine o = affine_from_xyzz(g1_scalar_mul(g, s));
+        NOTE_IDENTITY_BASE(flags, o.is_identity());
+        affine_store(out + 64 * i, o);
+    }
+}
+
+}
diff --git a/halo2-snark-aggregator_amd/csrc/fp.hpp b/halo2-snark-aggregator_amd/csrc/fp.hpp
--- a/halo2-snark-aggregator_amd/csrc/fp.hpp
+++ b/halo2-snark-aggregator_amd/csrc/fp.hpp
@@ -117,6 +117,34 @@
 #pragma unroll
     for (int i = 0; i < NL; ++i) x[i] = (int32_t)km_limb<P>(K, i) - (int32_t)a.l[i];
     return fp_normalize<P>(x);
+}
+
+template <int KP, int KN, class P>
+FP_INLINE Fp<P> fp_sub_sgn(const Fp<P>& a, uint32_t sgn, const Fp<P>& b) {
+    int32_t x[NL];
+#pragma unroll
+    for (int i = 0; i < NL; ++i)
+        x[i] = (int32_t)((a.l[i] ^ sgn) + km_limb<P>(KP, i) + (sgn & (km_limb<P>(KN, i) + 1u - km_limb<P>(KP, i)))) - (int32_t)b.l[i];
+    return fp_normalize<P>(x);
+}
+
+template <class P>
+constexpr uint32_t km_limb_borrowed(int K, int i) {
+    return km_limb<P>(K, i) + (i < 8 ? (1u << 29) : 0u) - (i > 0 ? 1u : 0u);
+}
+template <int K, class P>
+FP_INLINE Fp<P> fp_sub_loose(const Fp<P>& a, const Fp<P>& b) {
+    Fp<P> r;
+#pragma unroll
+    for (int i = 0; i < NL; ++i) r.l[i] = a.l[i] + km_limb_borrowed<P>(K, i) - b.l[i];
+    return r;
+}
+template <int K, class P>
+FP_INLINE Fp<P> fp_neg_loose(const Fp<P>& a) {
+    Fp<P> r;
+#pragma unroll
+    for (int i = 0; i < NL; ++i) r.l[i] = km_limb_borrowed<P>(K, i) - a.l[i];
+    return r;
 }
 
 template <class P>
diff --git a/halo2-snark-aggregator_amd/csrc/h2agg.hip b/halo2-snark-aggregator_amd/csrc/h2agg.hip
--- a/halo2-snark-aggregator_amd/csrc/h2agg.hip
+++ b/halo2-snark-aggregator_amd/csrc/h2agg.hip
@@ -80,6 +80,7 @@
     uint8_t* d = nullptr;
     uint8_t* endo_x = nullptr;
     size_t n = 0;
+    bool no_identity = false;
     uint8_t* pre = nullptr;
     int pre_c = 0, pre_W = 0;
     uint8_t* comb = nullptr;
@@ -152,6 +153,9 @@
     int comm_rank = 0, comm_size = 0;
 
     int dbg_pcie_slices = 0, dbg_pcie_glv = 0, dbg_pcie_chain = 1, dbg_comb_msm = 1, dbg_plan_cache = 1, dbg_small_sort = 1, dbg_eval_split = 1, dbg_pre_big = 0, dbg_lean_acc = 1, dbg_shard_fail = 0, dbg_shard_calls = 0, dbg_phases = 0, dbg_tape_lds = 1, dbg_prewake = 1;
+    int dbg_lean_full = 0;
+    uint32_t table_word = 0;
+    int last_lean_variant = -1;
     int dbg_seg_chunk = 0, dbg_seg_c = 0;
     DevBuf seg_wsum, seg_dev, seg_out;
     DevBuf fft_tw[2], fft_scale;
@@ -277,6 +281,7 @@
     HIP_TRY(c, hipStreamSynchronize(c->stream));
     uint32_t f[3];
     memcpy(f, c->h_pinned + 2048, 12);
+    c->table_word = f[1];
     f[0] |= host_flags;
     if (f[0] | f[2]) HIP_TRY(c, hipMemsetAsync(c->d_flags, 0, 12, c->stream));
     if (f[0]) return flags_to_status(c, f[0], false);
@@ -493,8 +498,31 @@
     return !c->cfg_no_dm && !c->cfg_no_stage && !c->cfg_stage_l1 && !c->cfg_sub_bits && !c->cfg_tile && !c->cfg_seg;
 }
 
+int msm_lean_variant(bool table_no_identity, bool plan_glv) {
+    return (table_no_identity ? 0 : LEAN_ID) | (plan_glv ? LEAN_ENDO : 0);
+}
+bool table_word_clear(uint32_t word) { return word == 0; }
+
+using AccLeanKernel = decltype(&k_msm_accumulate_lean<0, true>);
+template <bool DUAL>
+AccLeanKernel acc_lean_kernel(int chain, int var) {
+    const int ch = chain == CHAIN_FIRST ? 1 : (chain == CHAIN_MID || chain == CHAIN_LAST) ? 2 : 0;
+#define ACC_LEAN_ROW(CH)                                                                                      \
+    case CH:                                                                                                   \
+        return var == 0 ? k_msm_accumulate_lean_v<CH, DUAL, 0> : var == LEAN_ID ? k_msm_accumulate_lean_v<CH, DUAL, LEAN_ID> \
+             : var == LEAN_ENDO ? k_msm_accumulate_lean_v<CH, DUAL, LEAN_ENDO> : k_msm_accumulate_lean<CH, DUAL>;
+    switch (ch) {
+        ACC_LEAN_ROW(1)
+        ACC_LEAN_ROW(2)
+        default:
+        ACC_LEAN_ROW(0)
+    }
+#undef ACC_LEAN_ROW
+}
+
 int msm_run(h2agg_ctx* c, const uint8_t* d_bases, const uint8_t* d_scalars, size_t n_base, uint8_t* d_out_jac,
-            uint32_t batch = 1, const uint8_t* d_endo_x = nullptr, const PreTable* pre = nullptr, uint32_t split = 0) {
+            uint32_t batch = 1, const uint8_t* d_endo_x = nullptr, const PreTable* pre = nullptr, uint32_t split = 0,
+            bool no_identity = false) {
     if (split) batch = 2;
     const size_t n = split ? n_base : n_base * batch;
     crumb((uintptr_t)__builtin_return_address(0), ((uint64_t)batch << 40) | n_base);
@@ -842,11 +870,13 @@
         if (lean) {
 #ifdef H2AGG_MEASURE_KNOBS
             static const bool lean_dual = !(knob("H2AGG_ACC") && !strcmp(knob("H2AGG_ACC"), "lean1"));
-            auto kacc = lean_dual ? (chain == CHAIN_FIRST ? k_msm_accumulate_lean<1, true> : (chain == CHAIN_MID || chain == CHAIN_LAST) ? k_msm_accumulate_lean<2, true> : k_msm_accumulate_lean<0, true>)
-                                  : (chain == CHAIN_FIRST ? k_msm_accumulate_lean<1, false> : (chain == CHAIN_MID || chain == CHAIN_LAST) ? k_msm_accumulate_lean<2, false> : k_msm_accumulate_lean<0, false>);
+            const int var = msm_lean_variant(no_identity && !c->dbg_lean_full, p.glv || c->dbg_lean_full);
+            auto kacc = lean_dual ? acc_lean_kernel<true>(chain, var) : acc_lean_kernel<false>(chain, var);
 #else
-            auto kacc = chain == CHAIN_FIRST ? k_msm_accumulate_lean<1, true> : (chain == CHAIN_MID || chain == CHAIN_LAST) ? k_msm_accumulate_lean<2, true> : k_msm_accumulate_lean<0, true>;
+            const int var = msm_lean_variant(no_identity && !c->dbg_lean_full, p.glv || c->dbg_lean_full);
+            auto kacc = acc_lean_kernel<true>(chain, var);
 #endif
+            c->last_lean_variant = var;
             hipLaunchKernelGGL(kacc, dim3((unsigned)(((size_t)p.NBT * lpb + 63) / 64)), dim3(64), (size_t)acc_lds,
                                st, d_bases, d_endo_x, entries, offs, hist, ordered ? order : (uint32_t*)nullptr, p.NBT, p.big, lpb, acc_out,
                                big_list, big_keys, big_count, fix_list);
@@ -1503,6 +1533,7 @@
         hipFree(t.d);
         return rc;
     }
+    t.no_identity = table_word_clear(c->table_word);
     uint64_t h = c->next_handle++;
     c->tables[h] = t;
     *handle_out = h;
@@ -1553,6 +1584,7 @@
         hipFree(t.d);
         return rc;
     }
+    t.no_identity = table_word_clear(c->table_word);
     uint64_t h = c->next_handle++;
     c->tables[h] = t;
     *handle_out = h;
@@ -1725,7 +1757,8 @@
             return msm_run(c, it->second.d, (const uint8_t*)d_scalars, n, (uint8_t*)d_out_jac, 1, nullptr, &pt);
     }
     const size_t SLICE = (size_t)1 << 22;
-    if (n <= SLICE) return msm_run(c, it->second.d, (const uint8_t*)d_scalars, n, (uint8_t*)d_out_jac, 1, endo);
+    const bool no_id = it->second.no_identity;
+    if (n <= SLICE) return msm_run(c, it->second.d, (const uint8_t*)d_scalars, n, (uint8_t*)d_out_jac, 1, endo, nullptr, 0, no_id);
     const size_t nsl = (n + SLICE - 1) / SLICE;
     const bool was_overlap = c->tail_overlap;
     const int was_level = c->overlap_level;
@@ -1737,7 +1770,8 @@
     for (size_t k = 0; k < nsl && rc == H2AGG_OK; ++k) {
         const size_t off = k * SLICE, m = n - off < SLICE ? n - off : SLICE;
         c->chain = k == 0 ? CHAIN_FIRST : (k + 1 == nsl ? CHAIN_LAST : CHAIN_MID);
-        rc = msm_run(c, it->second.d + 64 * off, (const uint8_t*)d_scalars + 32 * off, m, (uint8_t*)d_out_jac, 1, endo + 32 * off);
+        rc = msm_run(c, it->second.d + 64 * off, (const uint8_t*)d_scalars + 32 * off, m, (uint8_t*)d_out_jac, 1, endo + 32 * off,
+                     nullptr, 0, no_id);
     }
     c->chain = CHAIN_OFF;
     c->tail_overlap = was_overlap;
@@ -1792,7 +1826,7 @@
     for (size_t q = 0; q < batch && rc == H2AGG_OK; q += per) {
         const size_t b = batch - q < per ? batch - q : per;
         rc = msm_run(c, it->second.d, (const uint8_t*)d_scalars + 32 * n * q, n, (uint8_t*)d_out_jac + 96 * q, (uint32_t)b,
-                     use_pre ? nullptr : endo, use_pre ? &pt : nullptr);
+                     use_pre ? nullptr : endo, use_pre ? &pt : nullptr, 0, !use_pre && it->second.no_identity);
     }
     c->tail_overlap = was_overlap;
     c->overlap_level = was_level;
@@ -2125,8 +2159,26 @@
         if (value != 0 && (value < (int)LK_TILE_LOG_MIN || value > (int)LK_TILE_LOG)) return fail(c, H2AGG_ERR_INVALID, "h2agg_debug_configure: fr_sort_tile must be 0 or 4 .. 11");
         c->dbg_fr_sort_tile = value;
     }
+    else if (k == "lean_full") c->dbg_lean_full = value;
     else if (k == "pre_big") c->dbg_pre_big = value;
     else return fail(c, H2AGG_ERR_INVALID, "h2agg_debug_configure: unknown key " + k);
+    return H2AGG_OK;
+} catch (...) {
+    return H2AGG_ERR_INVALID;
+}
+
+int h2agg_debug_lean_variant(int table_no_identity, int plan_glv) {
+    return msm_lean_variant(table_no_identity != 0, plan_glv != 0);
+}
+
+int h2agg_debug_table_identity(h2agg_ctx* c, uint64_t handle, int* may_hold_out, int* last_variant_out) try {
+    TRY(bind(c));
+    if (may_hold_out) {
+        auto it = c->tables.find(handle);
+        if (it == c->tables.end()) return fail(c, H2AGG_ERR_INVALID, "unknown base-table handle");
+        *may_hold_out = it->second.no_identity ? 0 : 1;
+    }
+    if (last_variant_out) *last_variant_out = c->last_lean_variant;
     return H2AGG_OK;
 } catch (...) {
     return H2AGG_ERR_INVALID;
diff --git a/halo2-snark-aggregator_amd/csrc/msm_kernels.hpp b/halo2-snark-aggregator_amd/csrc/msm_kernels.hpp
--- a/halo2-snark-aggregator_amd/csrc/msm_kernels.hpp
+++ b/halo2-snark-aggregator_amd/csrc/msm_kernels.hpp
@@ -130,23 +130,30 @@
 }
 
 struct RawPt { uint4 a, b, c, d; };
+constexpr int LEAN_ID = 1, LEAN_ENDO = 2;
+template <int VAR>
 FP_INLINE RawPt raw_gather(const uint8_t* __restrict__ bases, const uint8_t* __restrict__ endo_x, uint32_t e) {
     const size_t idx = e & ENT_IDX;
-    const uint4* px = reinterpret_cast<const uint4*>((e & ENT_ENDO) ? endo_x + 32 * idx : bases + 64 * idx);
+    const uint4* px = reinterpret_cast<const uint4*>(((VAR & LEAN_ENDO) && (e & ENT_ENDO)) ? endo_x + 32 * idx : bases + 64 * idx);
     const uint4* py = reinterpret_cast<const uint4*>(bases + 64 * idx + 32);
     RawPt r;
     r.a = px[0]; r.b = px[1]; r.c = py[0]; r.d = py[1];
     return r;
 }
-FP_INLINE G1Affine raw_unpack(const RawPt& r, uint32_t e) {
+FP_INLINE G1Affine raw_unpack(const RawPt& r) {
     G1Affine p;
     { uint32_t w[8] = {r.a.x, r.a.y, r.a.z, r.a.w, r.b.x, r.b.y, r.b.z, r.b.w}; p.x = fp_unpack<FqParams>(w); }
     { uint32_t w[8] = {r.c.x, r.c.y, r.c.z, r.c.w, r.d.x, r.d.y, r.d.z, r.d.w}; p.y = fp_unpack<FqParams>(w); }
-    return (e & ENT_NEG) ? affine_neg(p) : p;
-}
-template <bool DUAL, class NextF>
-FP_INLINE bool xyzz_add_affine_lean(G1XYZZ& acc, G1Affine q, NextF&& issue_next) {
-    bool ok = !q.is_identity() && !acc.is_identity();
+    return p;
+}
+FP_INLINE uint32_t ent_sign(uint32_t e) {
+    static_assert(ENT_NEG == 0x80000000u, "the sign is the entry's top bit");
+    return (uint32_t)((int32_t)e >> 31);
+}
+template <bool DUAL, int VAR, class NextF>
+FP_INLINE bool xyzz_add_affine_lean(G1XYZZ& acc, G1Affine q, uint32_t sgn, NextF&& issue_next) {
+    bool ok = true;
+    if (VAR & LEAN_ID) ok = !q.is_identity();
     if (DUAL) {
         fpa_mul_dual_ip<FqParams>(q.x, acc.zz, q.y, acc.zzz);
     } else {
@@ -154,7 +161,7 @@
         fpa_mul_ip<FqParams>(q.y, acc.zzz);
     }
     Fq p = FQ_SUB(8, q.x, acc.x);
-    Fq r = FQ_SUB(4, q.y, acc.y);
+    Fq r = fp_sub_sgn<4, 6, FqParams>(q.y, sgn, acc.y);
     ok = ok && !fp_maybe_zero_mod2<10, FqParams>(p);
     if (!ok) return false;
     Fq pp, rr;
@@ -168,9 +175,9 @@
         fpa_mul_ip<FqParams>(acc.x, pp);
     }
     Fq x3 = fp_sub_sub2<6, FqParams>(rr, p, acc.x);
-    Fq d = FQ_SUB(8, acc.x, x3);
+    Fq d = fp_sub_loose<10, FqParams>(acc.x, x3);
     acc.x = x3;
-    Fq ny = fp_neg<4, FqParams>(acc.y);
+    Fq ny = fp_neg_loose<8, FqParams>(acc.y);
     if (DUAL) {
         fpa_mul_dual_ip<FqParams>(acc.zz, pp, acc.zzz, p);
         issue_next();
@@ -183,11 +190,11 @@
     acc.y = ny;
     return true;
 }
-template <bool DUAL>
-FP_INLINE bool xyzz_add_affine_affine_lean(G1XYZZ& o, const G1Affine& a, const G1Affine& q) {
+template <bool DUAL, int VAR>
+FP_INLINE bool xyzz_add_affine_affine_lean(G1XYZZ& o, const G1Affine& a, const G1Affine& q, uint32_t sgn) {
     Fq p = FQ_SUB(2, q.x, a.x);
-    Fq r = FQ_SUB(2, q.y, a.y);
-    if (q.is_identity() || fp_maybe_zero_mod2<4, FqParams>(p)) return false;
+    Fq r = fp_sub_sgn<2, 4, FqParams>(q.y, sgn, a.y);
+    if (((VAR & LEAN_ID) && q.is_identity()) || fp_maybe_zero_mod2<4, FqParams>(p)) return false;
     Fq pp, rr;
     Fq qq = a.x;
     if (DUAL) {
@@ -200,8 +207,8 @@
         fpa_mul_ip<FqParams>(qq, pp);
     }
     o.x = fp_sub_sub2<6, FqParams>(rr, p, qq);
-    Fq d = FQ_SUB(8, qq, o.x);
-    Fq ny = fp_neg<2, FqParams>(a.y);
+    Fq d = fp_sub_loose<10, FqParams>(qq, o.x);
+    Fq ny = fp_neg_loose<4, FqParams>(a.y);
     if (DUAL) fpa_mul2_ip<FqParams>(ny, p, r, d);
     else fpa_mul2_ip1<FqParams>(ny, p, r, d);
     o.y = ny;
@@ -210,13 +217,13 @@
     return true;
 }
 
-template <int CHAIN, bool DUAL>
-__global__ void __launch_bounds__(64) __attribute__((amdgpu_waves_per_eu(4, 4)))
-k_msm_accumulate_lean(const uint8_t* __restrict__ bases, const uint8_t* __restrict__ endo_x,
-                      const uint32_t* __restrict__ entries, const uint32_t* __restrict__ offs,
-                      const uint32_t* __restrict__ hist, const uint32_t* __restrict__ order, uint32_t nbt, uint32_t big,
-                      uint32_t lpb, uint8_t* __restrict__ buckets, uint32_t* __restrict__ big_list,
-                      uint32_t* __restrict__ big_keys, uint32_t* __restrict__ counters, uint32_t* __restrict__ fix_list) {
+template <int CHAIN, bool DUAL, int VAR>
+FP_INLINE void msm_accumulate_lean_body(const uint8_t* __restrict__ bases, const uint8_t* __restrict__ endo_x,
+                                        const uint32_t* __restrict__ entries, const uint32_t* __restrict__ offs,
+                                        const uint32_t* __restrict__ hist, const uint32_t* __restrict__ order, uint32_t nbt,
+                                        uint32_t big, uint32_t lpb, uint8_t* __restrict__ buckets,
+                                        uint32_t* __restrict__ big_list, uint32_t* __restrict__ big_keys,
+                                        uint32_t* __restrict__ counters, uint32_t* __restrict__ fix_list) {
     const uint32_t t = blockIdx.x * blockDim.x + threadIdx.x;
     if (t >= nbt * lpb) return;
     const uint32_t part = t % lpb;
@@ -255,25 +262,27 @@
     uint32_t k = lo;
     if (hi > lo) {
         uint32_t e_cur = run(lo);
-        RawPt nxt = raw_gather(bases, endo_x, e_cur);
+        RawPt nxt = raw_gather<VAR>(bases, endo_x, e_cur);
         uint32_t e_nxt = run(lo + 1 < hi ? lo + 1 : hi - 1);
         auto advance = [&](uint32_t k_now) {
             e_cur = e_nxt;
-            nxt = raw_gather(bases, endo_x, e_nxt);
+            nxt = raw_gather<VAR>(bases, endo_x, e_nxt);
             e_nxt = run(k_now + 2 < hi ? k_now + 2 : hi - 1);
         };
         bool go = true;
-        if (acc.is_identity()) {
-            const G1Affine first = raw_unpack(nxt, e_cur);
+        if (CHAIN != 2 || acc.is_identity()) {
+            G1Affine first = raw_unpack(nxt);
             go = !first.is_identity();
             if (go) {
+                if (e_cur & ENT_NEG) first.y = fp_neg<2, FqParams>(first.y);
                 advance(lo);
                 k = lo + 1;
                 acc = G1XYZZ::from_affine(first);
                 if (k < hi) {
-                    const G1Affine second = raw_unpack(nxt, e_cur);
+                    const G1Affine second = raw_unpack(nxt);
+                    const uint32_t sgn = ent_sign(e_cur);
                     advance(lo + 1);
-                    go = xyzz_add_affine_affine_lean<DUAL>(acc, first, second);
+                    go = xyzz_add_affine_affine_lean<DUAL, VAR>(acc, first, second, sgn);
                     if (go) k = lo + 2;
                 }
             }
@@ -281,8 +290,9 @@
         if (go) {
 #pragma unroll 1
             for (; k < hi; ++k) {
-                const G1Affine cur = raw_unpack(nxt, e_cur);
-                if (!xyzz_add_affine_lean<DUAL>(acc, cur, [&]() { advance(k); })) break;
+                const G1Affine cur = raw_unpack(nxt);
+                const uint32_t sgn = ent_sign(e_cur);
+                if (!xyzz_add_affine_lean<DUAL, VAR>(acc, cur, sgn, [&]() { advance(k); })) break;
             }
         }
         if (k < hi) {
@@ -295,6 +305,23 @@
     asm volatile("" : "+v"(oslot));
     xyzz_store(buckets + XYZZ_BYTES * (size_t)oslot, acc);
 }
+#define MSM_ACC_LEAN_PARAMS                                                                                              \
+    const uint8_t *__restrict__ bases, const uint8_t *__restrict__ endo_x, const uint32_t *__restrict__ entries,         \
+        const uint32_t *__restrict__ offs, const uint32_t *__restrict__ hist, const uint32_t *__restrict__ order,        \
+        uint32_t nbt, uint32_t big, uint32_t lpb, uint8_t *__restrict__ buckets, uint32_t *__restrict__ big_list,        \
+        uint32_t *__restrict__ big_keys, uint32_t *__restrict__ counters, uint32_t *__restrict__ fix_list
+#define MSM_ACC_LEAN_ARGS bases, endo_x, entries, offs, hist, order, nbt, big, lpb, buckets, big_list, big_keys, counters, fix_list
+template <int CHAIN, bool DUAL>
+__global__ void __launch_bounds__(64) __attribute__((amdgpu_waves_per_eu(4, 4))) k_msm_accumulate_lean(MSM_ACC_LEAN_PARAMS) {
+    msm_accumulate_lean_body<CHAIN, DUAL, LEAN_ID | LEAN_ENDO>(MSM_ACC_LEAN_ARGS);
+}
+template <int CHAIN, bool DUAL, int VAR>
+__global__ void __launch_bounds__(64) __attribute__((amdgpu_waves_per_eu(4, 4))) k_msm_accumulate_lean_v(MSM_ACC_LEAN_PARAMS) {
+    static_assert(VAR >= 0 && VAR < (LEAN_ID | LEAN_ENDO), "the full set is k_msm_accumulate_lean");
+    msm_accumulate_lean_body<CHAIN, DUAL, VAR>(MSM_ACC_LEAN_ARGS);
+}
+#undef MSM_ACC_LEAN_PARAMS
+#undef MSM_ACC_LEAN_ARGS
 __global__ void __launch_bounds__(64) k_msm_accumulate_fix(const uint8_t* __restrict__ bases, const uint8_t* __restrict__ endo_x,
                                                            const uint32_t* __restrict__ entries,
                                                            const uint32_t* __restrict__ offs,
diff --git a/halo2-snark-aggregator_amd/csrc/params.inc b/halo2-snark-aggregator_amd/csrc/params.inc
--- a/halo2-snark-aggregator_amd/csrc/params.inc
+++ b/halo2-snark-aggregator_amd/csrc/params.inc
@@ -145,6 +145,7 @@
         hipFree(t.d);
         return rc;
     }
+    t.no_identity = table_word_clear(c->table_word);
     const uint64_t h = c->next_handle++;
     c->tables[h] = t;
     *out_handle = h;
@@ -182,6 +183,7 @@
         if (tl.d) hipFree(tl.d);
         return rc;
     }
+    tg.no_identity = tl.no_identity = table_word_clear(c->table_word);
     if (tg.d) {
         const uint64_t h = c->next_handle++;
         c->tables[h] = tg;
diff --git a/halo2-snark-aggregator_amd/csrc/scalar_mul_kernels.hpp b/halo2-snark-aggregator_amd/csrc/scalar_mul_kernels.hpp
--- a/halo2-snark-aggregator_amd/csrc/scalar_mul_kernels.hpp
+++ b/halo2-snark-aggregator_amd/csrc/scalar_mul_kernels.hpp
@@ -179,7 +179,9 @@
             const uint32_t d = (s.w[w >> 2] >> (8 * (w & 3))) & 0xffu;
             if (d) xyzz_add_affine(acc, affine_load(table + 64 * ((size_t)w * COMB_ROW + d - 1)));
         }
-        affine_store(out + 64 * i, affine_from_xyzz(acc));
+        const G1Affine o = affine_from_xyzz(acc);
+        NOTE_IDENTITY_BASE(flags, o.is_identity());
+        affine_store(out + 64 * i, o);
     }
 }
 
diff --git a/include/h2agg.h b/include/h2agg.h
--- a/include/h2agg.h
+++ b/include/h2agg.h
@@ -246,6 +246,8 @@
 int h2agg_msm_configure_lanes_per_bucket(h2agg_ctx* ctx, int lanes);
 int h2agg_msm_configure_sort(h2agg_ctx* ctx, int sub_bits, int tile);
 int h2agg_debug_configure(h2agg_ctx* ctx, const char* key, int value);
+int h2agg_debug_lean_variant(int table_no_identity, int plan_glv);
+int h2agg_debug_table_identity(h2agg_ctx* ctx, uint64_t handle, int* may_hold_out, int* last_variant_out);
 int h2agg_msm_set_tail_overlap(h2agg_ctx* ctx, int enable);
 int h2agg_profile_enable(h2agg_ctx* ctx, int enable);
 int h2agg_profile_reset(h2agg_ctx* ctx);
```

Result: faster. 849.6 million (median of 6 runs) (+1.7%).
